# theEricMa/ScaleDreamer

Hardware: AMD Instinct MI355X
Metric: ASD train steps/sec (64x64 render, SD2.1) (higher is better)
Workload: dtype f32 renderer / f16 diffusion (f32 accumulate); 1 GPU; asd_sd_nerf: 1 view/GPU, 64x64 rays, 512 spp occgrid march, implicit-volume iNGP (16x2 hash grid 2^19, MLP 64), SD-2.1 UNet batch 5 (CFG+Perp-Neg+shifted t), VAE 512^2 fwd+bwd, AdamW; views_per_gpu=1, parallelism=dp1, diffusion_backend=hip, diffusion_weights=seeded random init (seed 1)

## Files before the change

### scaledreamer_amd/csrc/asd_common.h

```cpp
#pragma once
#include <hip/hip_runtime.h>
#include <stdint.h>

#include "../../include/asd_hip.h"

#define ASD_WAVE 64

void asd_set_error(const char* fmt, ...);

#define ASD_CHECK_ARG(cond, msg)                          \
    do {                                                  \
        if (!(cond)) {                                    \
            asd_set_error("%s: %s", __func__, msg);       \
            return ASD_ERR_ARG;                           \
        }                                                 \
    } while (0)

#define ASD_LAUNCH_CHECK()                                                         \
    do {                                                                           \
        hipError_t e__ = hipGetLastError();                                        \
        if (e__ != hipSuccess) {                                                   \
            asd_set_error("%s: launch failed: %s", __func__, hipGetErrorString(e__)); \
            return ASD_ERR_LAUNCH;                                                 \
        }                                                                          \
    } while (0)

static inline int asd_div_up(int64_t a, int64_t b) { return (int)((a + b - 1) / b); }

#include <atomic>
static inline bool asd_attr_needed(std::atomic<unsigned long long>& mask) {
    int dev = 0;
    (void)hipGetDevice(&dev);
    const unsigned long long bit = 1ull << (dev & 63);
    if (mask.load(std::memory_order_relaxed) & bit) return false;
    mask.fetch_or(bit, std::memory_order_relaxed);
    return true;
}

static inline int asd_grid_for(int64_t n, int block) {
    int g = asd_div_up(n, block);
    if (g < 1) g = 1;
    if (g > 2048) g = 2048;
    return g;
}

#ifdef __HIPCC__
__device__ __forceinline__ int asd_lane() { return (int)(threadIdx.x & 63); }

__device__ __forceinline__ float asd_wave_sum(float v) {
    int x;
#define ASD_DPP_ADD(CTRL, ROW_MASK)                                                                                      \
    x = __builtin_amdgcn_update_dpp(0, __float_as_int(v), CTRL, ROW_MASK, 0xf, true);                                    \
    v += __int_as_float(x)
    ASD_DPP_ADD(0x111, 0xf);
    ASD_DPP_ADD(0x112, 0xf);
    ASD_DPP_ADD(0x114, 0xf);
    ASD_DPP_ADD(0x118, 0xf);
    ASD_DPP_ADD(0x142, 0xa);
    ASD_DPP_ADD(0x143, 0xc);
#undef ASD_DPP_ADD
    return __int_as_float(__builtin_amdgcn_readlane(__float_as_int(v), 63));
}

__device__ __forceinline__ float asd_row_sum15(float v) {
    int x;
#define ASD_DPP_ADD(CTRL)                                                                                                \
    x = __builtin_amdgcn_update_dpp(0, __float_as_int(v), CTRL, 0xf, 0xf, true);                                         \
    v += __int_as_float(x)
    ASD_DPP_ADD(0x111);
    ASD_DPP_ADD(0x112);
    ASD_DPP_ADD(0x114);
    ASD_DPP_ADD(0x118);
#undef ASD_DPP_ADD
    return v;
}

__device__ __forceinline__ float asd_wave_incl_scan(float v) {
    const int lane = asd_lane();
#pragma unroll
    for (int o = 1; o < 64; o <<= 1) {
        const float u = __shfl_up(v, o, 64);
        if (lane >= o) v += u;
    }
    return v;
}
__device__ __forceinline__ float asd_wave_incl_prod(float v) {
    const int lane = asd_lane();
#pragma unroll
    for (int o = 1; o < 64; o <<= 1) {
        const float u = __shfl_up(v, o, 64);
        if (lane >= o) v *= u;
    }
    return v;
}
__device__ __forceinline__ int asd_ballot_rank(unsigned long long mask) {
    return (int)__builtin_amdgcn_mbcnt_hi((unsigned)(mask >> 32), __builtin_amdgcn_mbcnt_lo((unsigned)mask, 0u));
}

__device__ __forceinline__ float asd_softplus(float x) { return x > 20.f ? x : log1pf(expf(x)); }
__device__ __forceinline__ float asd_sigmoid(float x) { return 1.f / (1.f + expf(-x)); }
__device__ __forceinline__ float asd_clampf(float v, float lo, float hi) { return v < lo ? lo : (v > hi ? hi : v); }

__device__ __forceinline__ uint32_t asd_grid_index(const asd_grid_meta& m, int l, uint32_t cx, uint32_t cy,
                                                   uint32_t cz) {
    const uint32_t res = m.resolution[l];
    const uint32_t size = m.size[l];
    uint32_t di = cx + cy * res + cz * res * res;
    di -= (di >= size) ? size : 0u;
    const uint32_t hi = ((cx * 1u) ^ (cy * 2654435761u) ^ (cz * 805459861u)) & (size - 1u);
    return m.dense[l] ? di : hi;
}
__device__ __forceinline__ float asd_unit(float x) { return fminf(fmaxf(x, 0.f), 1.f); }

template <int L>
__device__ __forceinline__ void asd_encode(const asd_grid_meta& m, const float* __restrict__ params, float x,
                                           float y, float z, float (&enc)[2 * L]) {
    x = asd_unit(x); y = asd_unit(y); z = asd_unit(z);
#pragma unroll
    for (int l = 0; l < L; ++l) {
        const float s = m.scale[l];
        const float px = fmaf(s, x, 0.5f), py = fmaf(s, y, 0.5f), pz = fmaf(s, z, 0.5f);
        const float fx = floorf(px), fy = floorf(py), fz = floorf(pz);
        const uint32_t cx = (uint32_t)(int32_t)fx, cy = (uint32_t)(int32_t)fy, cz = (uint32_t)(int32_t)fz;
        const float wx = px - fx, wy = py - fy, wz = pz - fz;
        const float2* __restrict__ tab = reinterpret_cast<const float2*>(params) + m.offset[l];
        float2 v[8];
#pragma unroll
        for (int c = 0; c < 8; ++c)
            v[c] = tab[asd_grid_index(m, l, cx + (c & 1), cy + ((c >> 1) & 1), cz + ((c >> 2) & 1))];
        float f0 = 0.f, f1 = 0.f;
#pragma unroll
        for (int c = 0; c < 8; ++c) {
            const float ax = (c & 1) ? wx : 1.f - wx;
            const float ay = (c & 2) ? wy : 1.f - wy;
            const float az = (c & 4) ? wz : 1.f - wz;
            const float wt = ax * ay * az;
            f0 = fmaf(wt, v[c].x, f0);
            f1 = fmaf(wt, v[c].y, f1);
        }
        enc[2 * l] = f0;
        enc[2 * l + 1] = f1;
        if ((l & 3) == 3) __builtin_amdgcn_sched_barrier(0);
    }
}

template <int L>
__device__ __forceinline__ void asd_scatter(const asd_grid_meta& m, float* __restrict__ dparams, float x, float y,
                                            float z, const float (&denc)[2 * L]) {
    x = asd_unit(x); y = asd_unit(y); z = asd_unit(z);
#pragma unroll
    for (int l = 0; l < L; ++l) {
        const float g0 = denc[2 * l], g1 = denc[2 * l + 1];
        if (g0 == 0.f && g1 == 0.f) continue;
        const float s = m.scale[l];
        const float px = fmaf(s, x, 0.5f), py = fmaf(s, y, 0.5f), pz = fmaf(s, z, 0.5f);
        const float fx = floorf(px), fy = floorf(py), fz = floorf(pz);
        const uint32_t cx = (uint32_t)(int32_t)fx, cy = (uint32_t)(int32_t)fy, cz = (uint32_t)(int32_t)fz;
        const float wx = px - fx, wy = py - fy, wz = pz - fz;
        float* __restrict__ tab = dparams + 2u * (size_t)m.offset[l];
#pragma unroll
        for (int c = 0; c < 8; ++c) {
            const float ax = (c & 1) ? wx : 1.f - wx;
            const float ay = (c & 2) ? wy : 1.f - wy;
            const float az = (c & 4) ? wz : 1.f - wz;
            const float wt = ax * ay * az;
            const uint32_t idx = asd_grid_index(m, l, cx + (c & 1), cy + ((c >> 1) & 1), cz + ((c >> 2) & 1));
            atomicAdd(tab + 2u * (size_t)idx, wt * g0);
            atomicAdd(tab + 2u * (size_t)idx + 1, wt * g1);
        }
    }
}
#ifndef ASD_PRIV_COPIES
#define ASD_PRIV_COPIES 8
#endif
template <int L, int NAGG, int NPRIV = 0, bool FINE = true>
__device__ __forceinline__ void asd_scatter_runs(const asd_grid_meta& m, float* __restrict__ dparams, float x, float y,
                                                 float z, const float (&denc)[2 * L], bool active, float* __restrict__ priv = nullptr,
                                                 uint32_t priv_stride = 0) {
    static_assert(NPRIV <= NAGG, "only run-aggregated levels have per-XCD copies");
    x = asd_unit(x); y = asd_unit(y); z = asd_unit(z);
    const int lane = asd_lane();
    if (NPRIV > 0) {
        unsigned xcc, copy;
        asm volatile("s_getreg_b32 %0, hwreg(HW_REG_XCC_ID)" : "=s"(xcc));
        copy = xcc & 7u;
        if (ASD_PRIV_COPIES > 8) {
            unsigned hwid;
            asm volatile("s_getreg_b32 %0, hwreg(HW_REG_HW_ID)" : "=s"(hwid));
            copy = copy * (ASD_PRIV_COPIES / 8) + ((hwid >> 8) & (ASD_PRIV_COPIES / 8 - 1));
        }
        priv += (size_t)copy * priv_stride;
    }
#pragma unroll
    for (int l = 0; l < (NAGG < L ? NAGG : L); ++l) {
        const float g0 = active ? denc[2 * l] : 0.f, g1 = active ? denc[2 * l + 1] : 0.f;
        const float s = m.scale[l];
        const float px = fmaf(s, x, 0.5f), py = fmaf(s, y, 0.5f), pz = fmaf(s, z, 0.5f);
        const float fx = floorf(px), fy = floorf(py), fz = floorf(pz);
        const uint32_t cx = (uint32_t)(int32_t)fx, cy = (uint32_t)(int32_t)fy, cz = (uint32_t)(int32_t)fz;
        const float wx = px - fx, wy = py - fy, wz = pz - fz;
        float* __restrict__ tab = (l < NPRIV ? priv : dparams) + 2u * (size_t)m.offset[l];
        const uint32_t res = m.resolution[l];
        const uint32_t key = active ? cx + (cy + cz * res) * res : 0xFFFFFFFFu - (uint32_t)lane;
        const uint32_t prev = __shfl_up(key, 1, 64);
        const bool head = lane == 0 || prev != key;
        const unsigned long long hm = __ballot(head);
        const int rid = __popcll(hm & (~0ull >> (63 - lane)));
        float v[16];
#pragma unroll
        for (int c = 0; c < 8; ++c) {
            const float wt = ((c & 1) ? wx : 1.f - wx) * ((c & 2) ? wy : 1.f - wy) * ((c & 4) ? wz : 1.f - wz);
            v[2 * c] = wt * g0;
            v[2 * c + 1] = wt * g1;
        }
#pragma unroll
        for (int o = 1; o < 64; o <<= 1) {
            const int prid = __shfl_down(rid, o, 64);
            const bool ok = (lane + o < 64) && prid == rid;
#pragma unroll
            for (int q = 0; q < 16; ++q) {
                const float u = __shfl_down(v[q], o, 64);
                v[q] += ok ? u : 0.f;
            }
        }
        const bool issue = head && active;
        const bool carrier = !head && ((hm >> (lane - 1)) & 1ull);
        const bool self_f1 = issue && (lane == 63 || ((hm >> (lane + 1)) & 1ull));
#pragma unroll
        for (int c = 0; c < 8; ++c) {
            const uint32_t idx = asd_grid_index(m, l, cx + (c & 1), cy + ((c >> 1) & 1), cz + ((c >> 2) & 1));
            const float f1_prev = __shfl_up(v[2 * c + 1], 1, 64);
            const float val = issue ? v[2 * c] : f1_prev;
            float* dst = tab + 2u * (size_t)idx + (issue ? 0 : 1);
            if ((issue || carrier) && val != 0.f) atomicAdd(dst, val);
            if (self_f1 && v[2 * c + 1] != 0.f) atomicAdd(tab + 2u * (size_t)idx + 1, v[2 * c + 1]);
        }
    }
    if (NAGG >= L || !FINE) return;
    const int xb = (lane >> 1) & 1, ft = lane & 1;
#pragma unroll 1
    for (int q = 0; q < 4; ++q) {
        const int src = 16 * q + (lane >> 2);
        const float sx = __shfl(x, src, 64), sy = __shfl(y, src, 64), sz = __shfl(z, src, 64);
        const bool sact = __shfl((int)active, src, 64) != 0;
#pragma unroll
        for (int l = (NAGG < L ? NAGG : L); l < L; ++l) {
            const float ga = __shfl(denc[2 * l], src, 64), gb = __shfl(denc[2 * l + 1], src, 64);
            const float g = ft ? gb : ga;
            if (!sact || g == 0.f) continue;
            const float s = m.scale[l];
            const float px = fmaf(s, sx, 0.5f), py = fmaf(s, sy, 0.5f), pz = fmaf(s, sz, 0.5f);
            const float fx = floorf(px), fy = floorf(py), fz = floorf(pz);
            const uint32_t cx = (uint32_t)(int32_t)fx + (uint32_t)xb, cy = (uint32_t)(int32_t)fy, cz = (uint32_t)(int32_t)fz;
            const float wx = px - fx, wy = py - fy, wz = pz - fz;
            const float ax = xb ? wx : 1.f - wx;
            float* __restrict__ tab = dparams + 2u * (size_t)m.offset[l] + ft;
#pragma unroll
            for (int c = 0; c < 4; ++c) {
                const float wt = ax * ((c & 1) ? wy : 1.f - wy) * ((c & 2) ? wz : 1.f - wz);
                const uint32_t idx = asd_grid_index(m, l, cx, cy + (c & 1), cz + ((c >> 1) & 1));
                atomicAdd(tab + 2u * (size_t)idx, wt * g);
            }
        }
    }
}

extern hipEvent_t g_asd_probe_start, g_asd_probe_stop;
#define ASD_PROBE_START(s) do { if (g_asd_probe_start) (void)hipEventRecord(g_asd_probe_start, (s)); } while (0)
#define ASD_PROBE_STOP(s) do { if (g_asd_probe_stop) (void)hipEventRecord(g_asd_probe_stop, (s)); } while (0)

#endif
```

### scaledreamer_amd/csrc/gemm.hip

```cpp
#include <stdlib.h>

#include "asd_common.h"
#include <map>
#include <atomic>
#include <mutex>
#include <cstring>
#include <iterator>

#include "gemm_tile.h"


template <int BM, int BN, int WM, int WN, bool CONV, int NST = 2, int KG = 1, bool LN = false>
__global__ __launch_bounds__(WM * WN * KG * 64) void gemm_f16_kernel(const asd_gemm_args p) {
    constexpr int NW = WM * WN;
    constexpr int TM = BM / WM / 16, TN = BN / WN / 16;
    constexpr int RB = 128;
    constexpr int A_BYTES = BM * RB, B_BYTES = BN * RB;
    constexpr int STAGE_BYTES = A_BYTES + B_BYTES;
    constexpr int ASLABS = BM / 8, TSLABS = (BM + BN) / 8;
    constexpr int SPW = (TSLABS + NW - 1) / NW;
    static_assert(BM % (WM * 16) == 0 && BN % (WN * 16) == 0, "wave tile must be a multiple of 16 x 16");
    static_assert(NST == 2 || TSLABS % NW == 0, "ring variants count their loads per wave: every wave must own the same number of slabs");
    static_assert(KG == 1 || NST == 2, "k-groups use the two-stage loop");
    extern __shared__ __attribute__((aligned(16))) char smem[];

    const int tid = threadIdx.x, lane = tid & 63;
    const int wave_all = __builtin_amdgcn_readfirstlane(tid >> 6);
    const int kg = KG > 1 ? wave_all / NW : 0;
    const int wave = wave_all - kg * NW;
    char* const gsm = smem + kg * (NST * STAGE_BYTES);
    const int wm = wave / WN, wn = wave % WN;
    const bool up3 = CONV && p.upsample == 3;
    const int up_mq = up3 ? p.M >> 2 : 1;
    const int tiles_pp = (up_mq + BM - 1) / BM;
    const int tiles_m = up3 ? 4 * tiles_pp : (p.M + BM - 1) / BM, tiles_n = (p.N + BN - 1) / BN;
    int item, tm_, tn_;
    if (!asd_xcd_item(blockIdx.x, tiles_m * tiles_n * p.split_k, item)) return;
    const int kz = item / (tiles_m * tiles_n);
    asd_grouped_tile(item - kz * tiles_m * tiles_n, tiles_m, tiles_n, p.group_m, p.group_n, tm_, tn_);
    const int parity = up3 ? tm_ / tiles_pp : 0;
    const int m0 = up3 ? parity * up_mq + (tm_ - parity * tiles_pp) * BM : tm_ * BM, n0 = tn_ * BN;
    const int m_lim = up3 ? (parity + 1) * up_mq : p.M;
    const int k_steps_total = (p.K + 63) / 64;
    const int k_per = (k_steps_total + p.split_k - 1) / p.split_k;
    const int ks0 = kz * k_per, ks1 = min(k_steps_total, ks0 + k_per);

    const int lrow = lane >> 3, pchunk = lane & 7;
    const char* zero = (const char*)p.zero_page;
    const bool fast_conv = CONV && (p.upsample == 0 || p.upsample == 3) && (p.Cin & 63) == 0;
    const int par_a = parity >> 1, par_b = parity & 1;
    const char* const Wp = (const char*)p.W + ((CONV && p.upsample == 3) ? (size_t)parity * p.N * p.ldw * 2 : 0);
    const int lch = pchunk ^ lrow;
    constexpr int ASPW = (ASLABS + NW - 1) / NW;
    const char* a0 = nullptr;
    const char* c_base[CONV ? ASPW : 1];
    int c_yx[CONV ? ASPW : 1];
    if (!CONV) {
        a0 = (const char*)p.A + (size_t)(m0 + lrow) * p.lda * 2 + lch * 16;
    } else {
#pragma unroll
        for (int j = 0; j < ASPW; ++j) {
            const int slab = wave + j * NW;
            int m = min(m0 + slab * 8 + lrow, m_lim - 1);
            int hw = p.Hout * p.Wout, wrow = p.Wout;
            if (p.upsample == 3) { m -= parity * up_mq; hw = p.Hin * p.Win; wrow = p.Win; }
            const int b = m / hw, r = m - b * hw;
            int y = r / wrow, x = r - y * wrow;
            c_base[j] = (const char*)p.A + (size_t)b * p.Hin * p.Win * p.Cin * 2;
            if (fast_conv) {
                y *= p.stride; x *= p.stride;
                c_base[j] += ((size_t)(y * p.Win + x) * p.Cin) * 2 + lch * 16;
            }
            c_yx[j] = (y << 16) | x;
        }
    }
    constexpr bool WIDE_OK = (BN / WN) % 32 == 0;
    const bool wide = WIDE_OK && p.wide_rows;
    const int wl = wide ? wide_lane_row(lrow) : lrow;
    auto w_slab_rows = [&](int ws) { return wide ? wide_slab_rows(ws) : ws * 8; };
    const char* w0 = Wp + (size_t)(n0 + wl) * p.ldw * 2 + lch * 16;
    const size_t a_slab_stride = (size_t)8 * p.lda * 2, w_row_stride = (size_t)p.ldw * 2;
    unsigned roff[SPW];
#pragma unroll
    for (int j = 0; j < SPW; ++j) {
        const int slab = wave + j * NW;
        if (slab >= ASLABS) {
            const int row = min(n0 + w_slab_rows(slab - ASLABS) + wl, p.N - 1);
            roff[j] = (unsigned)row * (unsigned)(p.ldw * 2) + lch * 16 + (ks0 + kg) * 128;
            if (!CONV && p.w_seg_rows > 0) {
                const int seg = row / p.w_seg_rows;
                roff[j] = (unsigned)(row - seg * p.w_seg_rows) * (unsigned)(p.ldw * 2) + (unsigned)p.w_seg_off[seg] + lch * 16 + (ks0 + kg) * 128;
            }
        } else {
            const int row = min(m0 + slab * 8 + lrow, p.M - 1);
            roff[j] = CONV ? 0u : (unsigned)row * (unsigned)(p.lda * 2) + lch * 16 + (ks0 + kg) * 128;
            if (!CONV && p.a_seg_rows > 0) {
                const int seg = row / p.a_seg_rows;
                roff[j] = (unsigned)(row - seg * p.a_seg_rows) * (unsigned)(p.lda * 2) + (unsigned)p.a_seg_off[seg] + lch * 16 + (ks0 + kg) * 128;
            }
        }
    }

    auto issue_rows = [&](int stage) __attribute__((always_inline)) {
        char* st = gsm + stage * STAGE_BYTES;
#pragma unroll
        for (int j = 0; j < SPW; ++j) {
            const int slab = wave + j * NW;
            if (j * NW + NW - 1 >= TSLABS && slab >= TSLABS) continue;
            if (CONV && slab < ASLABS) continue;
            const char* base = slab >= ASLABS ? Wp : (const char*)p.A;
            load_slab(base + roff[j], st + slab * 8 * RB);
            roff[j] += 128 * KG;
        }
    };
    auto issue_general = [&](int ks, int stage, bool only_conv_a) __attribute__((always_inline)) {
        char* st = gsm + stage * STAGE_BYTES;
        const int k0 = ks * 64;
        const int kc = k0 + lch * 8;
        const bool k_ok = kc < p.K;
        int opaque = 0;
        asm volatile("" : "+v"(opaque));
        int tdy = 0, tdx = 0;
        long long toff = 0;
        if (fast_conv) {
            const int tap = k0 / p.Cin, c0 = k0 - tap * p.Cin;
            if (p.upsample == 3) { tdy = (tap >> 1) - 1 + par_a; tdx = (tap & 1) - 1 + par_b; }
            else { const int ky = tap / 3, kx = tap - ky * 3; tdy = ky - p.pad; tdx = kx - p.pad; }
            toff = ((long long)(tdy * p.Win + tdx) * p.Cin + c0) * 2;
        }
#pragma unroll
        for (int j = 0; j < SPW; ++j) {
            const int slab = wave + j * NW;
            if (slab >= TSLABS) continue;
            if (only_conv_a && slab >= ASLABS) continue;
            const char* src;
            if (slab >= ASLABS) {
                const int ws = slab - ASLABS;
                const int wr = w_slab_rows(ws);
                src = (k_ok && n0 + wr + wl < p.N) ? w0 + (wr + opaque) * w_row_stride + (size_t)k0 * 2 : zero;
            } else if (!CONV) {
                src = (k_ok && m0 + slab * 8 + lrow < p.M) ? a0 + (slab + opaque) * a_slab_stride + (size_t)k0 * 2 : zero;
            } else {
                constexpr int JA = CONV ? ASPW : 1;
                const int ja = j < JA ? j : JA - 1;
                const bool row_ok = m0 + slab * 8 + lrow < m_lim;
                const int sy = c_yx[ja] >> 16, sx = c_yx[ja] & 0xffff;
                if (fast_conv) {
                    const int yi = sy + tdy, xi = sx + tdx;
                    const bool ok = row_ok && (unsigned)yi < (unsigned)p.Hin && (unsigned)xi < (unsigned)p.Win;
                    src = ok ? c_base[ja] + toff : zero;
                } else {
                    const int tap = kc / p.Cin, c0 = kc - tap * p.Cin;
                    const int ky = tap / 3, kx = tap - ky * 3;
                    int yi = sy * p.stride + ky - p.pad, xi = sx * p.stride + kx - p.pad;
                    bool ok = row_ok && k_ok;
                    if (p.upsample == 3) {
                        yi = sy + (tap >> 1) - 1 + par_a; xi = sx + (tap & 1) - 1 + par_b;
                        ok = ok && yi >= 0 && xi >= 0 && yi < p.Hin && xi < p.Win;
                    } else if (p.upsample == 1) {
                        ok = ok && yi >= 0 && xi >= 0 && yi < 2 * p.Hin && xi < 2 * p.Win;
                        yi >>= 1; xi >>= 1;
                    } else if (p.upsample == 2) {
                        yi = sy + p.pad - ky; xi = sx + p.pad - kx;
                        ok = ok && yi >= 0 && xi >= 0 && !(yi & 1) && !(xi & 1) && (yi >> 1) < p.Hin && (xi >> 1) < p.Win;
                        yi >>= 1; xi >>= 1;
                    } else {
                        ok = ok && yi >= 0 && xi >= 0 && yi < p.Hin && xi < p.Win;
                    }
                    src = ok ? c_base[ja] + ((size_t)(yi * p.Win + xi) * p.Cin + c0) * 2 : zero;
                }
            }
            load_slab(src, st + slab * 8 * RB);
        }
    };
    auto issue = [&](int ks, int stage) __attribute__((always_inline)) {
        if (ks * 64 + 64 > p.K || (CONV && !fast_conv)) {
            issue_general(ks, stage, false);
        } else {
            issue_rows(stage);
            if (CONV) issue_general(ks, stage, true);
        }
    };

    floatx4 acc[TM][TN];
#pragma unroll
    for (int i = 0; i < TM; ++i)
#pragma unroll
        for (int j = 0; j < TN; ++j) acc[i][j] = floatx4{0.f, 0.f, 0.f, 0.f};
    floatx4 sacc[LN ? TM : 1], qacc[LN ? TM : 1];
#pragma unroll
    for (int i = 0; i < (LN ? TM : 1); ++i) sacc[i] = qacc[i] = floatx4{0.f, 0.f, 0.f, 0.f};
    const half8 ln_ones = {(half_t)1.f, (half_t)1.f, (half_t)1.f, (half_t)1.f, (half_t)1.f, (half_t)1.f, (half_t)1.f, (half_t)1.f};
    float ls1[LN ? TM : 1], ls2[LN ? TM : 1];
    auto ln_extract = [&]() __attribute__((always_inline)) {
        if constexpr (LN) {
            const int b = lane & 15;
#pragma unroll
            for (int i = 0; i < TM; ++i) {
                ls1[i] = sacc[i][0];
                const float d = (b & 2) ? ((b & 1) ? qacc[i][3] : qacc[i][2]) : ((b & 1) ? qacc[i][1] : qacc[i][0]);
                ls2[i] = __shfl(d, b + 16 * (b >> 2), 64);
            }
        }
    };

    const int frow = lane & 15, fq = lane >> 4;
    const int fa0 = (wm * (BM / WM) + frow) * RB, fb0 = A_BYTES + (wn * (BN / WN) + frow) * RB;
    const int fsw[2] = {((fq) ^ (frow & 7)) * 16, ((4 + fq) ^ (frow & 7)) * 16};

    int live_ky_parity = -1;
    if (NST == 2 && KG == 1 && CONV && p.upsample == 2 && (p.Cin & 63) == 0) {
        const int m_last = min(m0 + BM, p.M) - 1;
        if (m0 / p.Wout == m_last / p.Wout) live_ky_parity = ((m0 / p.Wout) % p.Hout + p.pad) & 1;
    }
    auto live = [&](int ks) -> bool {
        if (!CONV || live_ky_parity < 0) return true;
        const int ky = ((ks * 64) / p.Cin) / 3;
        return (ky & 1) == live_ky_parity;
    };
    auto compute = [&](const char* As) __attribute__((always_inline)) {
#pragma unroll TM * TN >= 32 ? 1 : 2
        for (int kh = 0; kh < 2; ++kh) {
            half8 xa[TM], wb[TN];
            const int fs = TM * TN >= 32 ? (((kh * 4 + fq) ^ (frow & 7)) * 16) : fsw[kh];
#pragma unroll
            for (int i = 0; i < TM; ++i) xa[i] = *(const half8*)(As + fa0 + fs + i * 16 * RB);
#pragma unroll
            for (int j = 0; j < TN; ++j) wb[j] = *(const half8*)(As + fb0 + fs + j * 16 * RB);
#pragma unroll
            for (int i = 0; i < TM; ++i)
#pragma unroll
                for (int j = 0; j < TN; ++j)
                    acc[i][j] = __builtin_amdgcn_mfma_f32_16x16x32_f16(wb[j], xa[i], acc[i][j], 0, 0, 0);
            if constexpr (LN) {
#pragma unroll
                for (int i = 0; i < TM; ++i) {
                    sacc[i] = __builtin_amdgcn_mfma_f32_16x16x32_f16(ln_ones, xa[i], sacc[i], 0, 0, 0);
                    qacc[i] = __builtin_amdgcn_mfma_f32_16x16x32_f16(xa[i], xa[i], qacc[i], 0, 0, 0);
                }
            }
        }
    };
    if constexpr (KG > 1) {
        int k = ks0 + kg;
        const int iters = (ks1 - ks0 + KG - 1) / KG;
        if (k < ks1) issue(k, 0);
        for (int it = 0, stage = 0; it < iters; ++it, stage ^= 1) {
            asm volatile("s_waitcnt vmcnt(0)" ::: "memory");
            __builtin_amdgcn_s_barrier();
            const int kn = k + KG;
            if (kn < ks1) issue(kn, stage ^ 1);
            if (k < ks1) compute(gsm + stage * STAGE_BYTES);
            k = kn;
        }
        ln_extract();
        floatx4* red = (floatx4*)smem;
#pragma unroll 1
        for (int g = KG - 1; g >= 1; --g) {
            __syncthreads();
            if (kg == g) {
#pragma unroll
                for (int i = 0; i < TM; ++i)
#pragma unroll
                    for (int j = 0; j < TN; ++j) red[((wave * TM + i) * TN + j) * 64 + lane] = acc[i][j];
            }
            __syncthreads();
            if (kg == 0) {
#pragma unroll
                for (int i = 0; i < TM; ++i)
#pragma unroll
                    for (int j = 0; j < TN; ++j) {
                        const floatx4 t = red[((wave * TM + i) * TN + j) * 64 + lane];
                        acc[i][j][0] += t[0]; acc[i][j][1] += t[1]; acc[i][j][2] += t[2]; acc[i][j][3] += t[3];
                    }
            }
            if constexpr (LN) {
                float* redf = (float*)(red + NW * TM * TN * 64);
                __syncthreads();
                if (kg == g) {
#pragma unroll
                    for (int i = 0; i < TM; ++i) { redf[((wave * TM + i) * 2) * 64 + lane] = ls1[i]; redf[((wave * TM + i) * 2 + 1) * 64 + lane] = ls2[i]; }
                }
                __syncthreads();
                if (kg == 0) {
#pragma unroll
                    for (int i = 0; i < TM; ++i) { ls1[i] += redf[((wave * TM + i) * 2) * 64 + lane]; ls2[i] += redf[((wave * TM + i) * 2 + 1) * 64 + lane]; }
                }
            }
        }
    } else if constexpr (NST > 2) {
        const int nk = ks1 - ks0;
        if (nk > 0) {
#pragma unroll
            for (int s = 0; s < NST - 1; ++s)
                if (s < nk) issue(ks0 + s, s);
            int stage = 0, fill = NST - 1;
            for (int i = 0; i < nk; ++i) {
                ring_wait<SPW, NST - 2>(nk - 1 - i);
                __builtin_amdgcn_s_barrier();
                if (i + NST - 1 < nk) issue(ks0 + i + NST - 1, fill);
                compute(gsm + stage * STAGE_BYTES);
                stage = stage + 1 == NST ? 0 : stage + 1;
                fill = fill + 1 == NST ? 0 : fill + 1;
            }
        }
    } else {
    int k = ks0;
    while (k < ks1 && !live(k)) ++k;
    if (k < ks1) {
        issue(k, 0);
        for (int stage = 0;; stage ^= 1) {
            asm volatile("s_waitcnt vmcnt(0)" ::: "memory");
            __builtin_amdgcn_s_barrier();
            int kn = k + 1;
            while (kn < ks1 && !live(kn)) ++kn;
            if (kn < ks1) issue(kn, stage ^ 1);
            compute(gsm + stage * STAGE_BYTES);
            if (kn >= ks1) break;
            k = kn;
        }
    }
    }
    if constexpr (KG == 1) ln_extract();

    const int em = lane & 15, en = (lane >> 4) * 4;
    auto out_row = [&](int i) {
        const int m = m0 + wm * (BM / WM) + i * 16 + em;
        if (m >= m_lim) return -1;
        if (CONV && p.upsample == 3) {
            const int q = m - parity * up_mq, hwq = p.Hin * p.Win;
            const int bb = q / hwq, r = q - bb * hwq, y = r / p.Win, x = r - y * p.Win;
            return (bb * p.Hout + 2 * y + par_a) * p.Wout + 2 * x + par_b;
        }
        return m;
    };
    if (KG > 1 && kg != 0) {
        if (p.split_k == 1 && p.act != 2 && p.gn_partials != nullptr) {
            __syncthreads(); __syncthreads();
            __syncthreads();
        }
        return;
    }
    if (p.split_k > 1) {
        tile_epilogue<TM, TN>(p, acc, n0 + wn * (BN / WN), kz, m0, out_row, false, nullptr);
        return;
    }
    float ln_mean[LN ? TM : 1], ln_rstd[LN ? TM : 1];
    if constexpr (LN) {
        const float inv_k = 1.f / (float)p.K;
#pragma unroll
        for (int i = 0; i < TM; ++i) {
            ln_mean[i] = ls1[i] * inv_k;
            ln_rstd[i] = rsqrtf(fmaxf(ls2[i] * inv_k - ln_mean[i] * ln_mean[i], 0.f) + p.ln_eps);
            const int m = m0 + wm * (BM / WM) + i * 16 + em;
            if (p.ln_stats && n0 == 0 && wn == 0 && lane < 16 && m < p.M) { p.ln_stats[2 * m] = ln_mean[i]; p.ln_stats[2 * m + 1] = ln_rstd[i]; }
        }
    }
    if (p.act == 2) {
        if constexpr (TN % 2 == 0) {
#pragma unroll
            for (int i = 0; i < TM; ++i) {
                const int m = m0 + wm * (BM / WM) + i * 16 + em;
                if (m >= p.M) continue;
#pragma unroll
                for (int j = 0; j < TN; j += 2) {
                    const int n = n0 + wn * (BN / WN) + j * 16 + en;
                    if (n + 16 >= p.N) continue;
                    const half4 bx = *(const half4*)((const half_t*)p.bias + n), bg = *(const half4*)((const half_t*)p.bias + n + 16);
                    float va[4] = {acc[i][j][0], acc[i][j][1], acc[i][j][2], acc[i][j][3]};
                    float vg[4] = {acc[i][j + 1][0], acc[i][j + 1][1], acc[i][j + 1][2], acc[i][j + 1][3]};
                    if (p.ln_mode) {
                        ln_fold<4>(p, va, m, n, LN ? ln_mean[i] : 0.f, LN ? ln_rstd[i] : 0.f);
                        ln_fold<4>(p, vg, m, n + 16, LN ? ln_mean[i] : 0.f, LN ? ln_rstd[i] : 0.f);
                    }
                    half4 o;
#pragma unroll
                    for (int r = 0; r < 4; ++r)
                        o[r] = (half_t)((va[r] + (float)bx[r]) * gelu_erf(vg[r] + (float)bg[r]));
                    *(half4*)((half_t*)p.C + (size_t)m * p.ldc + (n >> 5) * 16 + (n & 15)) = o;
                }
            }
        }
        return;
    }
    const bool gn = p.gn_partials != nullptr;
    float* gn_lds = (float*)smem;
    if (gn) gn_tile_begin(gn_lds);
    tile_epilogue<TM, TN>(p, acc, n0 + wn * (BN / WN), kz, m0, out_row, gn, gn_lds, LN ? ln_mean : nullptr, LN ? ln_rstd : nullptr);
    if (gn) gn_tile_end(p, gn_lds, (m0 / BM) * ((p.N + BN - 1) / BN) + n0 / BN);
}

#define LDS_READ16(dst, addr, OFF) asm volatile("ds_read_b128 %0, %1 offset:%2" : "=&v"(dst) : "v"(addr), "n"(OFF) : "memory")
#define LGKM_WAIT(N, F)                                                                                                  \
    asm volatile("s_waitcnt lgkmcnt(" #N ")"                                                                             \
                 : "+v"(F.a[0]), "+v"(F.a[1]), "+v"(F.a[2]), "+v"(F.a[3]), "+v"(F.w[0]), "+v"(F.w[1]), "+v"(F.w[2]), "+v"(F.w[3]))

template <int BN>
__global__ __launch_bounds__(512) void conv3x3_win_kernel(const asd_gemm_args p) {
    constexpr int WN = 2, TM = 4, TN = BN / WN / 16;
    constexpr int RB = 128;
    constexpr int WIN = 18, WIN_ROWS = WIN * WIN, WIN_SLABS = (WIN_ROWS + 7) / 8;
    constexpr int A_BYTES = WIN_SLABS * 8 * RB, W_BYTES = BN * RB;
    constexpr int WSLABS = BN / 8, WSPW = (WSLABS + 7) / 8;
    extern __shared__ __attribute__((aligned(16))) char smem[];
    char* const a_buf = smem;
    char* const w_buf = smem + 2 * A_BYTES;

    const int tid = threadIdx.x, lane = tid & 63, wave = tid >> 6;
    const int wm = wave >> 1, wn = wave & 1;
    const int tiles_x = p.Wout / 16, tiles_y = p.Hout / 16;
    const int tiles_m = (p.M / (p.Hout * p.Wout)) * tiles_y * tiles_x;
    const int tiles_n = (p.N + BN - 1) / BN;
    int item, tm, tn_;
    if (!asd_xcd_item(blockIdx.x, tiles_m * tiles_n * p.split_k, item)) return;
    const int kz = item / (tiles_m * tiles_n);
    asd_grouped_tile(item - kz * tiles_m * tiles_n, tiles_m, tiles_n, p.group_m, p.group_n, tm, tn_);
    const int n0 = tn_ * BN;
    const int b = tm / (tiles_y * tiles_x), tr = tm - b * tiles_y * tiles_x;
    const int y0 = (tr / tiles_x) * 16, x0 = (tr - (tr / tiles_x) * tiles_x) * 16;
    const int n_chunks = p.Cin / 64;
    const int c_per = (n_chunks + p.split_k - 1) / p.split_k;
    const int c0 = kz * c_per, c1 = min(n_chunks, c0 + c_per);
    const int steps = (c1 - c0) * 9;

    const int lrow = lane >> 3, pchunk = lane & 7;
    const char* zero = (const char*)p.zero_page;
    const char* img = (const char*)p.A + (size_t)b * p.Hin * p.Win * p.Cin * 2;
    const bool wide = p.wide_rows != 0;
    const int wl = wide ? wide_lane_row(lrow) : lrow;
    const char* w0 = (const char*)p.W + (size_t)(n0 + wl) * p.ldw * 2 + (pchunk ^ lrow) * 16;
    const size_t w_row_stride = (size_t)p.ldw * 2;

    auto load_window_slab = [&](int slab, int chunk, char* dst_buf) {
        const int wrow = slab * 8 + lrow;
        const int wy = (wrow * 3641) >> 16, wx = wrow - wy * WIN;
        const int yi = y0 - 1 + wy, xi = x0 - 1 + wx;
        const bool ok = wrow < WIN_ROWS && (unsigned)yi < (unsigned)p.Hin && (unsigned)xi < (unsigned)p.Win;
        const char* src = ok ? img + ((size_t)(yi * p.Win + xi) * p.Cin + chunk * 64) * 2 + (pchunk ^ (wx & 7)) * 16 : zero;
        load_slab(src, dst_buf + slab * 8 * RB);
    };
    auto load_w_tile = [&](int step, char* dst_buf) {
        const int chunk = c0 + step / 9, tap = step - (step / 9) * 9;
        const size_t koff = ((size_t)tap * p.Cin + chunk * 64) * 2;
#pragma unroll
        for (int j = 0; j < WSPW; ++j) {
            const int slab = wave + j * 8;
            if (slab >= WSLABS) continue;
            const int wr = wide ? wide_slab_rows(slab) : slab * 8;
            const char* src = (n0 + wr + wl < p.N) ? w0 + wr * w_row_stride + koff : zero;
            load_slab(src, dst_buf + slab * 8 * RB);
        }
    };

    floatx4 acc[TM][TN];
#pragma unroll
    for (int i = 0; i < TM; ++i)
#pragma unroll
        for (int j = 0; j < TN; ++j) acc[i][j] = floatx4{0.f, 0.f, 0.f, 0.f};

    const int frow = lane & 15, fq = lane >> 4;
    const unsigned lds_a = (unsigned)(size_t)a_buf + (unsigned)((wm * 4 * WIN + frow) * RB);
    const unsigned lds_w = (unsigned)(size_t)w_buf + (unsigned)((wn * (BN / WN) + frow) * RB);
    const unsigned fsww[2] = {(unsigned)(((fq) ^ (frow & 7)) * 16), (unsigned)(((4 + fq) ^ (frow & 7)) * 16)};
    struct Frag { half8 a[4], w[4]; };
    static_assert(TM == 4 && (TN == 4 || TN == 2), "fragment sets are written for 4 x {2, 4} sub-tiles");

    auto read_frags = [&](Frag& f, int s, int kh) {
        const int cl = s / 9, tap = s - cl * 9;
        const int ky = tap / 3, kx = tap - ky * 3;
        const unsigned aa = lds_a + (unsigned)((cl & 1) * A_BYTES + (ky * WIN + kx) * RB) + (unsigned)(((kh * 4 + fq) ^ ((frow + kx) & 7)) * 16);
        const unsigned wa = lds_w + (unsigned)((s & 3) * W_BYTES) + fsww[kh];
        LDS_READ16(f.a[0], aa, 0 * WIN * RB);
        LDS_READ16(f.a[1], aa, 1 * WIN * RB);
        LDS_READ16(f.a[2], aa, 2 * WIN * RB);
        LDS_READ16(f.a[3], aa, 3 * WIN * RB);
        LDS_READ16(f.w[0], wa, 0 * 16 * RB);
        LDS_READ16(f.w[1], wa, 1 * 16 * RB);
        if constexpr (TN == 4) {
            LDS_READ16(f.w[2], wa, 2 * 16 * RB);
            LDS_READ16(f.w[3], wa, 3 * 16 * RB);
        } else {
            f.w[2] = f.w[0]; f.w[3] = f.w[1];
        }
    };
    auto mma = [&](const Frag& f) {
#pragma unroll
        for (int i = 0; i < TM; ++i)
#pragma unroll
            for (int j = 0; j < TN; ++j)
                acc[i][j] = __builtin_amdgcn_mfma_f32_16x16x32_f16(f.w[j], f.a[i], acc[i][j], 0, 0, 0);
    };
    constexpr int NRD = TM + TN;

    if (steps > 0) {
        for (int slab = wave; slab < WIN_SLABS; slab += 8) load_window_slab(slab, c0, a_buf);
        load_w_tile(0, w_buf);
        if (steps > 1) load_w_tile(1, w_buf + W_BYTES);
        Frag f0, f1;
#pragma unroll 1
        for (int s = 0; s < steps; s += 2) {
            const int cl = s / 9;
            asm volatile("s_waitcnt vmcnt(0)" ::: "memory");
            __builtin_amdgcn_s_barrier();
            if (s + 2 < steps) load_w_tile(s + 2, w_buf + ((s + 2) & 3) * W_BYTES);
            if (s + 3 < steps) load_w_tile(s + 3, w_buf + ((s + 3) & 3) * W_BYTES);
            if (c0 + cl + 1 < c1 && s > 9 * cl) {
                const int base = ((s - 9 * cl - 1) >> 1) * 16;
#pragma unroll
                for (int h = 0; h < 2; ++h) {
                    const int slab = base + h * 8 + wave;
                    if (slab < WIN_SLABS) load_window_slab(slab, c0 + cl + 1, a_buf + ((cl + 1) & 1) * A_BYTES);
                }
            }
            const bool two = s + 1 < steps;
            read_frags(f0, s, 0);
            read_frags(f1, s, 1);
            if constexpr (NRD == 8) LGKM_WAIT(8, f0); else LGKM_WAIT(6, f0);
            mma(f0);
            __builtin_amdgcn_sched_barrier(0);
            if (two) {
                read_frags(f0, s + 1, 0);
                if constexpr (NRD == 8) LGKM_WAIT(8, f1); else LGKM_WAIT(6, f1);
                mma(f1);
                __builtin_amdgcn_sched_barrier(0);
                read_frags(f1, s + 1, 1);
                if constexpr (NRD == 8) LGKM_WAIT(8, f0); else LGKM_WAIT(6, f0);
                mma(f0);
                __builtin_amdgcn_sched_barrier(0);
                LGKM_WAIT(0, f1);
                mma(f1);
            } else {
                LGKM_WAIT(0, f1);
                mma(f1);
            }
            __builtin_amdgcn_sched_barrier(0);
        }
    }

    const bool gn = p.gn_partials != nullptr && p.split_k == 1;
    float* gn_lds = (float*)smem;
    if (gn) gn_tile_begin(gn_lds);
    tile_epilogue<TM, TN>(p, acc, n0 + wn * (BN / WN), kz, b * p.Hout * p.Wout,
                          [&](int i) { return (b * p.Hout + y0 + wm * 4 + i) * p.Wout + x0 + frow; }, gn, gn_lds);
    if (gn) gn_tile_end(p, gn_lds, tm * tiles_n + tn_);
}

template <int BN, int NW = 8>
__global__ __launch_bounds__(NW * 64, NW / 2) void conv3x3_win2_kernel(const asd_gemm_args p) {
    constexpr int WN = NW / 4, TM = 4, TN = BN / WN / 16;
    constexpr int RB = 128;
    constexpr int WIN = 18, WIN_ROWS = WIN * WIN, WIN_SLABS = (WIN_ROWS + 7) / 8;
    constexpr int A_BYTES = WIN_SLABS * 8 * RB, W_BYTES = BN * RB;
    constexpr int WSLABS = BN / 8, WSPW = (WSLABS + NW - 1) / NW;
    extern __shared__ __attribute__((aligned(16))) char smem[];
    char* const a_buf = smem;
    char* const w_buf = smem + A_BYTES;

    const int tid = threadIdx.x, lane = tid & 63, wave = __builtin_amdgcn_readfirstlane(tid >> 6);
    const int wm = wave / WN, wn = wave - wm * WN;
    const int tiles_x = p.Wout / 16, tiles_y = p.Hout / 16;
    const int tiles_m = (p.M / (p.Hout * p.Wout)) * tiles_y * tiles_x;
    const int tiles_n = (p.N + BN - 1) / BN;
    int item, tm, tn_;
    if (!asd_xcd_item(blockIdx.x, tiles_m * tiles_n * p.split_k, item)) return;
    const int kz = item / (tiles_m * tiles_n);
    asd_grouped_tile(item - kz * tiles_m * tiles_n, tiles_m, tiles_n, p.group_m, p.group_n, tm, tn_);
    const int n0 = tn_ * BN;
    const int b = tm / (tiles_y * tiles_x), tr = tm - b * tiles_y * tiles_x;
    const int y0 = (tr / tiles_x) * 16, x0 = (tr - (tr / tiles_x) * tiles_x) * 16;
    const int n_chunks = p.Cin / 64;
    const int c_per = (n_chunks + p.split_k - 1) / p.split_k;
    const int c0 = kz * c_per, c1 = min(n_chunks, c0 + c_per);
    const int steps = (c1 - c0) * 9;

    const int lrow = lane >> 3, pchunk = lane & 7, lch = pchunk ^ lrow;
    const char* zero = (const char*)p.zero_page;
    const char* img = (const char*)p.A + (size_t)b * p.Hin * p.Win * p.Cin * 2;
    const bool wide = p.wide_rows != 0;
    const int wl = wide ? wide_lane_row(lrow) : lrow;
    const char* w0 = (const char*)p.W + (size_t)(n0 + wl) * p.ldw * 2 + lch * 16;
    const size_t w_row_stride = (size_t)p.ldw * 2;

    auto load_window_slab = [&](int slab, int chunk, char* dst_buf) {
        const int wrow = slab * 8 + lrow;
        const int wy = (wrow * 3641) >> 16, wx = wrow - wy * WIN;
        const int yi = y0 - 1 + wy, xi = x0 - 1 + wx;
        const bool ok = wrow < WIN_ROWS && (unsigned)yi < (unsigned)p.Hin && (unsigned)xi < (unsigned)p.Win;
        const char* src = ok ? img + ((size_t)(yi * p.Win + xi) * p.Cin + chunk * 64) * 2 + (pchunk ^ (wx & 7)) * 16 : zero;
        load_slab(src, dst_buf + slab * 8 * RB);
    };
    auto load_w_tile = [&](int step, char* dst_buf) {
        const int chunk = c0 + step / 9, tap = step - (step / 9) * 9;
        const size_t koff = ((size_t)tap * p.Cin + chunk * 64) * 2;
#pragma unroll
        for (int j = 0; j < WSPW; ++j) {
            const int slab = wave + j * NW;
            if (slab >= WSLABS) continue;
            const int wr = wide ? wide_slab_rows(slab) : slab * 8;
            const char* src = (n0 + wr + wl < p.N) ? w0 + wr * w_row_stride + koff : zero;
            load_slab(src, dst_buf + slab * 8 * RB);
        }
    };

    floatx4 acc[TM][TN];
#pragma unroll
    for (int i = 0; i < TM; ++i)
#pragma unroll
        for (int j = 0; j < TN; ++j) acc[i][j] = floatx4{0.f, 0.f, 0.f, 0.f};

    const int frow = lane & 15, fq = lane >> 4;
    const int fb0 = (wn * (BN / WN) + frow) * RB;
    const int fswb[2] = {((fq) ^ (frow & 7)) * 16, ((4 + fq) ^ (frow & 7)) * 16};

#ifdef ASD_WIN_PROFILE
    unsigned long long pt_start = __builtin_amdgcn_s_memtime(), pt_wait = 0, pt_first = 0, pt_reload = 0, pt_loop_end = 0;
#define PT_NOW() __builtin_amdgcn_s_memtime()
#endif
    if (steps > 0) {
        for (int slab = wave; slab < WIN_SLABS; slab += NW) load_window_slab(slab, c0, a_buf);
        load_w_tile(0, w_buf);
#pragma unroll 1
        for (int s = 0; s < steps; ++s) {
            const int cl = s / 9, tap = s - cl * 9;
#ifdef ASD_WIN_PROFILE
            const unsigned long long pt_a = PT_NOW();
#endif
            if (tap == 0 && s > 0) {
                __builtin_amdgcn_s_barrier();
                for (int slab = wave; slab < WIN_SLABS; slab += NW) load_window_slab(slab, c0 + cl, a_buf);
            }
            asm volatile("s_waitcnt vmcnt(0)" ::: "memory");
            __builtin_amdgcn_s_barrier();
#ifdef ASD_WIN_PROFILE
            {
                const unsigned long long pt_b = PT_NOW();
                if (s == 0) pt_first = pt_b - pt_a; else if (tap == 0) pt_reload += pt_b - pt_a; else pt_wait += pt_b - pt_a;
            }
#endif
            if (s + 1 < steps) load_w_tile(s + 1, w_buf + ((s + 1) & 1) * W_BYTES);
            const char* Wt = w_buf + (s & 1) * W_BYTES;
            const int ky = tap / 3, kx = tap - ky * 3;
            const char* Ar = a_buf + ((wm * 4 + ky) * WIN + frow + kx) * RB;
            const int csw = (frow + kx) & 7;
            if constexpr (NW == 4) {
                half8 xa[2][TM], wb[2][TN];
#pragma unroll
                for (int kh = 0; kh < 2; ++kh) {
                    const char* Ak = Ar + (((kh * 4 + fq) ^ csw) * 16);
#pragma unroll
                    for (int i = 0; i < TM; ++i) xa[kh][i] = *(const half8*)(Ak + i * WIN * RB);
#pragma unroll
                    for (int j = 0; j < TN; ++j) wb[kh][j] = *(const half8*)(Wt + fb0 + fswb[kh] + j * 16 * RB);
                }
                __builtin_amdgcn_sched_barrier(0);
#pragma unroll
                for (int kh = 0; kh < 2; ++kh)
#pragma unroll
                    for (int i = 0; i < TM; ++i)
#pragma unroll
                        for (int j = 0; j < TN; ++j)
                            acc[i][j] = __builtin_amdgcn_mfma_f32_16x16x32_f16(wb[kh][j], xa[kh][i], acc[i][j], 0, 0, 0);
            } else {
#pragma unroll
            for (int kh = 0; kh < 2; ++kh) {
                half8 xa[TM], wb[TN];
                const char* Ak = Ar + (((kh * 4 + fq) ^ csw) * 16);
#pragma unroll
                for (int i = 0; i < TM; ++i) xa[i] = *(const half8*)(Ak + i * WIN * RB);
#pragma unroll
                for (int j = 0; j < TN; ++j) wb[j] = *(const half8*)(Wt + fb0 + fswb[kh] + j * 16 * RB);
#pragma unroll
                for (int i = 0; i < TM; ++i)
#pragma unroll
                    for (int j = 0; j < TN; ++j)
                        acc[i][j] = __builtin_amdgcn_mfma_f32_16x16x32_f16(wb[j], xa[i], acc[i][j], 0, 0, 0);
            }
            }
        }
    }

#ifdef ASD_WIN_PROFILE
    pt_loop_end = PT_NOW();
#endif
    const bool gn = p.gn_partials != nullptr && p.split_k == 1;
    float* gn_lds = (float*)smem;
    if (gn) gn_tile_begin(gn_lds);
    tile_epilogue<TM, TN>(p, acc, n0 + wn * (BN / WN), kz, b * p.Hout * p.Wout,
                          [&](int i) { return (b * p.Hout + y0 + wm * 4 + i) * p.Wout + x0 + frow; }, gn, gn_lds);
    if (gn) gn_tile_end(p, gn_lds, tm * tiles_n + tn_);
#ifdef ASD_WIN_PROFILE
    if (p.split_k == 1 && p.workspace && lane == 0) {
        asm volatile("s_waitcnt vmcnt(0)" ::: "memory");
        unsigned long long* o = (unsigned long long*)p.workspace + ((size_t)item * NW + wave) * 8;
        o[0] = pt_start; o[1] = PT_NOW(); o[2] = pt_first; o[3] = pt_wait; o[4] = pt_reload; o[5] = pt_loop_end;
        unsigned hwid; asm volatile("s_getreg_b32 %0, hwreg(HW_REG_HW_ID)" : "=s"(hwid));
        unsigned xcc; asm volatile("s_getreg_b32 %0, hwreg(HW_REG_XCC_ID)" : "=s"(xcc));
        o[6] = hwid; o[7] = xcc;
    }
#endif
}

__global__ __launch_bounds__(256) void splitk_epilogue_kernel(const asd_gemm_args p, int splits) {
    const size_t q = (size_t)blockIdx.x * 256 + threadIdx.x;
    const size_t total4 = (size_t)p.M * p.N / 4;
    if (q >= total4) return;
    const int m = (int)((q * 4) / p.N), n = (int)((q * 4) % p.N);
    floatx4 v = {0.f, 0.f, 0.f, 0.f};
    for (int s = 0; s < splits; ++s) {
        const floatx4 t = *(const floatx4*)(p.workspace + ((size_t)s * p.M + m) * p.N + n);
        v[0] += t[0]; v[1] += t[1]; v[2] += t[2]; v[3] += t[3];
    }
    if (p.bias) {
        const half4 b = *(const half4*)((const half_t*)p.bias + n);
        v[0] += (float)b[0]; v[1] += (float)b[1]; v[2] += (float)b[2]; v[3] += (float)b[3];
    }
    if (p.row_bias) {
        const half4 b = *(const half4*)((const half_t*)p.row_bias + (size_t)(m / p.rows_per_group) * p.ld_row_bias + n);
        v[0] += (float)b[0]; v[1] += (float)b[1]; v[2] += (float)b[2]; v[3] += (float)b[3];
    }
    if (p.act == 1) {
#pragma unroll
        for (int r = 0; r < 4; ++r) v[r] = v[r] / (1.f + __expf(-v[r]));
    }
    if (p.residual) {
        const half4 b = *(const half4*)((const half_t*)p.residual + (size_t)m * p.ldr + n);
        v[0] += (float)b[0]; v[1] += (float)b[1]; v[2] += (float)b[2]; v[3] += (float)b[3];
    }
    if (p.out_f32) {
        *(floatx4*)((float*)p.C + (size_t)m * p.ldc + n) = v;
    } else {
        half4 o = {(half_t)v[0], (half_t)v[1], (half_t)v[2], (half_t)v[3]};
        *(half4*)((half_t*)p.C + (size_t)m * p.ldc + n) = o;
    }
}

__global__ __launch_bounds__(256) void splitk_epilogue_gn_kernel(const asd_gemm_args p, int splits) {
    __shared__ float lds64[64];
    const int tiles_n = p.N / 64;
    const int mb = blockIdx.x / tiles_n, nb = blockIdx.x - mb * tiles_n;
    const int tx = threadIdx.x & 15, ty = threadIdx.x >> 4;
    const int n = nb * 64 + tx * 4;
    if (threadIdx.x < 64) lds64[threadIdx.x] = 0.f;
    __syncthreads();
    floatx4 cs = {0.f, 0.f, 0.f, 0.f}, cq = {0.f, 0.f, 0.f, 0.f};
    half4 bias = {0, 0, 0, 0};
    if (p.bias) bias = *(const half4*)((const half_t*)p.bias + n);
    floatx4 v[4];
    int mrow[4];
#pragma unroll
    for (int i = 0; i < 4; ++i) {
        v[i] = floatx4{0.f, 0.f, 0.f, 0.f};
        mrow[i] = min(mb * 64 + i * 16 + ty, p.M - 1);
    }
    for (int s = 0; s < splits; ++s) {
        floatx4 t[4];
#pragma unroll
        for (int i = 0; i < 4; ++i) t[i] = *(const floatx4*)(p.workspace + ((size_t)s * p.M + mrow[i]) * p.N + n);
#pragma unroll
        for (int i = 0; i < 4; ++i) { v[i][0] += t[i][0]; v[i][1] += t[i][1]; v[i][2] += t[i][2]; v[i][3] += t[i][3]; }
    }
#pragma unroll
    for (int i = 0; i < 4; ++i) {
        const int m = mb * 64 + i * 16 + ty;
        if (m >= p.M) continue;
        floatx4 w = v[i];
        w[0] += (float)bias[0]; w[1] += (float)bias[1]; w[2] += (float)bias[2]; w[3] += (float)bias[3];
        if (p.row_bias) {
            const half4 b = *(const half4*)((const half_t*)p.row_bias + (size_t)(m / p.rows_per_group) * p.ld_row_bias + n);
            w[0] += (float)b[0]; w[1] += (float)b[1]; w[2] += (float)b[2]; w[3] += (float)b[3];
        }
        if (p.act == 1) {
#pragma unroll
            for (int r = 0; r < 4; ++r) w[r] = w[r] / (1.f + __expf(-w[r]));
        }
        if (p.residual) {
            const half4 b = *(const half4*)((const half_t*)p.residual + (size_t)m * p.ldr + n);
            w[0] += (float)b[0]; w[1] += (float)b[1]; w[2] += (float)b[2]; w[3] += (float)b[3];
        }
        const half4 o = {(half_t)w[0], (half_t)w[1], (half_t)w[2], (half_t)w[3]};
        *(half4*)((half_t*)p.C + (size_t)m * p.ldc + n) = o;
#pragma unroll
        for (int r = 0; r < 4; ++r) { const float f = (float)o[r]; cs[r] += f; cq[r] = fmaf(f, f, cq[r]); }
    }
#pragma unroll
    for (int r = 0; r < 4; ++r) {
        const int g = (n + r) / p.gn_cg;
        atomicAdd(&lds64[2 * g], cs[r]);
        atomicAdd(&lds64[2 * g + 1], cq[r]);
    }
    __syncthreads();
    if (threadIdx.x < 64) p.gn_partials[(size_t)blockIdx.x * 64 + threadIdx.x] = lds64[threadIdx.x];
}

#define GNA_THREADS 1024
template <int NV>
__global__ __launch_bounds__(GNA_THREADS) void splitk_epilogue_gnapply_kernel(const asd_gemm_args p, int splits) {
    __shared__ float red[2 * (GNA_THREADS / 64)];
    const int cg = p.gn_cg, g4 = cg >> 2, rows = p.gn_rows;
    const int b = blockIdx.x >> 5, g = blockIdx.x & 31;
    const int n0 = g * cg, total = rows * g4, tid = threadIdx.x;
    floatx4 v[NV];
    int mrow[NV], ncol[NV];
#pragma unroll
    for (int i = 0; i < NV; ++i) {
        const int e = min(tid + GNA_THREADS * i, total - 1);
        const int r = e / g4;
        mrow[i] = b * rows + r;
        ncol[i] = n0 + (e - r * g4) * 4;
        v[i] = floatx4{0.f, 0.f, 0.f, 0.f};
    }
    half4 bias[NV], rbias[NV], resid[NV];
#pragma unroll
    for (int i = 0; i < NV; ++i) {
        const int m = mrow[i], n = ncol[i];
        bias[i] = p.bias ? *(const half4*)((const half_t*)p.bias + n) : half4{0, 0, 0, 0};
        rbias[i] = p.row_bias ? *(const half4*)((const half_t*)p.row_bias + (size_t)(m / p.rows_per_group) * p.ld_row_bias + n) : half4{0, 0, 0, 0};
        resid[i] = p.residual ? *(const half4*)((const half_t*)p.residual + (size_t)m * p.ldr + n) : half4{0, 0, 0, 0};
    }
    for (int s = 0; s < splits; s += 4) {
        floatx4 t[4][NV];
#pragma unroll
        for (int u = 0; u < 4; ++u) {
            const int su = min(s + u, splits - 1);
#pragma unroll
            for (int i = 0; i < NV; ++i) t[u][i] = *(const floatx4*)(p.workspace + ((size_t)su * p.M + mrow[i]) * p.N + ncol[i]);
        }
#pragma unroll
        for (int u = 0; u < 4; ++u) {
            const float on = s + u < splits ? 1.f : 0.f;
#pragma unroll
            for (int i = 0; i < NV; ++i) {
                v[i][0] = fmaf(t[u][i][0], on, v[i][0]); v[i][1] = fmaf(t[u][i][1], on, v[i][1]);
                v[i][2] = fmaf(t[u][i][2], on, v[i][2]); v[i][3] = fmaf(t[u][i][3], on, v[i][3]);
            }
        }
    }
    float cs = 0.f, cq = 0.f;
#pragma unroll
    for (int i = 0; i < NV; ++i) {
        const int m = mrow[i], n = ncol[i];
        floatx4 w = v[i];
#pragma unroll
        for (int r = 0; r < 4; ++r) w[r] += (float)bias[i][r];
#pragma unroll
        for (int r = 0; r < 4; ++r) w[r] += (float)rbias[i][r];
        if (p.act == 1) {
#pragma unroll
            for (int r = 0; r < 4; ++r) w[r] = w[r] / (1.f + __expf(-w[r]));
        }
#pragma unroll
        for (int r = 0; r < 4; ++r) w[r] += (float)resid[i][r];
        const half4 o = {(half_t)w[0], (half_t)w[1], (half_t)w[2], (half_t)w[3]};
        const bool live = tid + GNA_THREADS * i < total;
        if (live) *(half4*)((half_t*)p.C + (size_t)m * p.ldc + n) = o;
#pragma unroll
        for (int r = 0; r < 4; ++r) {
            const float f = (float)o[r];
            v[i][r] = f;
            if (live) { cs += f; cq = fmaf(f, f, cq); }
        }
    }
#pragma unroll
    for (int off = 32; off > 0; off >>= 1) { cs += __shfl_xor(cs, off, 64); cq += __shfl_xor(cq, off, 64); }
    if ((tid & 63) == 0) { red[(tid >> 6) * 2] = cs; red[(tid >> 6) * 2 + 1] = cq; }
    __syncthreads();
    float sum = 0.f, sq = 0.f;
#pragma unroll
    for (int w = 0; w < GNA_THREADS / 64; ++w) { sum += red[2 * w]; sq += red[2 * w + 1]; }
    if (p.gn_apply_stats && tid == 0) { p.gn_apply_stats[b * 64 + g * 2] = sum; p.gn_apply_stats[b * 64 + g * 2 + 1] = sq; }
    const float inv_cnt = 1.f / ((float)rows * (float)cg);
    const float mean = sum * inv_cnt;
    const float var = fmaxf(sq * inv_cnt - mean * mean, 0.f);
    const float rstd = rsqrtf(var + p.gn_apply_eps);
#pragma unroll
    for (int i = 0; i < NV; ++i) {
        if (tid + GNA_THREADS * i >= total) continue;
        const int m = mrow[i], n = ncol[i];
        const half4 gm = *(const half4*)((const half_t*)p.gn_apply_gamma + n), bt = *(const half4*)((const half_t*)p.gn_apply_beta + n);
        half4 o;
#pragma unroll
        for (int r = 0; r < 4; ++r) {
            const float sa = rstd * (float)gm[r];
            float f = fmaf(v[i][r], sa, (float)bt[r] - mean * sa);
            if (p.gn_apply_silu) f = f / (1.f + __expf(-f));
            o[r] = (half_t)f;
        }
        *(half4*)((half_t*)p.gn_apply_y + (size_t)m * p.N + n) = o;
    }
}

#define ASD_GNAPPLY_MAX_NV 5
static int asd_gemm_gn_apply_nv(const asd_gemm_args* a) {
    if (!a->gn_apply || a->split_k <= 1 || a->partials_only || a->out_f32 || a->act == 2 || a->gn_bwd_x) return 0;
    if (a->gn_cg < 4 || a->gn_cg % 4 || a->N != 32 * a->gn_cg || a->gn_rows < 1 || a->M % a->gn_rows || a->ldc % 4) return 0;
    if (a->conv && a->upsample == 3) return 0;
    const int need = (a->gn_rows * (a->gn_cg / 4) + GNA_THREADS - 1) / GNA_THREADS;
    static const int max_nv = getenv("ASD_GNAPPLY_MAX_NV") ? atoi(getenv("ASD_GNAPPLY_MAX_NV")) : 3;
    if (need > max_nv) return 0;
    return need <= 1 ? 1 : need <= 3 ? 3 : need <= ASD_GNAPPLY_MAX_NV ? ASD_GNAPPLY_MAX_NV : 0;
}

static void asd_launch_splitk_epilogue(const asd_gemm_args* a, hipStream_t s) {
    const int nv = a->gn_apply_y ? asd_gemm_gn_apply_nv(a) : 0;
    if (nv > 0) {
        const dim3 grid((a->M / a->gn_rows) * 32);
        if (nv == 1) hipLaunchKernelGGL(splitk_epilogue_gnapply_kernel<1>, grid, dim3(GNA_THREADS), 0, s, *a, a->split_k);
        else if (nv == 3) hipLaunchKernelGGL(splitk_epilogue_gnapply_kernel<3>, grid, dim3(GNA_THREADS), 0, s, *a, a->split_k);
        else hipLaunchKernelGGL(splitk_epilogue_gnapply_kernel<ASD_GNAPPLY_MAX_NV>, grid, dim3(GNA_THREADS), 0, s, *a, a->split_k);
        return;
    }
    const size_t total4 = (size_t)a->M * a->N / 4;
    if (a->gn_partials) hipLaunchKernelGGL(splitk_epilogue_gn_kernel, dim3((a->M / 64) * (a->N / 64)), dim3(256), 0, s, *a, a->split_k);
    else hipLaunchKernelGGL(splitk_epilogue_kernel, dim3(asd_div_up(total4, 256)), dim3(256), 0, s, *a, a->split_k);
}


struct asd_gemm_tile { int bm, bn, wm, wn, nst, kg; };
#define ASD_GEMM_NCFG 29
#define ASD_GEMM_WIN0 8
#define ASD_GEMM_PP0 20
static const asd_gemm_tile asd_gemm_tiles[ASD_GEMM_NCFG] = {
    {128, 64, 2, 2}, {128, 128, 2, 2}, {256, 64, 4, 2}, {256, 128, 4, 2}, {128, 320, 2, 4}, {256, 256, 2, 4}, {256, 320, 2, 4},
    {320, 128, 5, 2}, {256, 64, 4, 2}, {256, 128, 4, 2}, {256, 64, 4, 2}, {256, 128, 4, 2},
    {64, 64, 2, 2},
    {256, 64, 4, 1}, {256, 128, 4, 1},
    {64, 64, 2, 2, 4, 1}, {64, 64, 2, 2, 2, 2}, {64, 64, 2, 2, 2, 4}, {128, 64, 2, 2, 2, 2}, {128, 128, 2, 2, 2, 2},
    {512, 128, 4, 2}, {256, 256, 4, 2}, {256, 320, 4, 2}, {256, 128, 4, 2}, {256, 160, 4, 2},
    {320, 64, 2, 2},
    {128, 64, 2, 2, 6, 1}, {64, 64, 2, 2, 8, 1}, {128, 128, 2, 2, 4, 1}};
#define ASD_GEMM_WS 25
static int asd_cfg_stages(int cfg) { return asd_gemm_tiles[cfg].nst > 2 ? asd_gemm_tiles[cfg].nst : 2; }
static int asd_cfg_kgroups(int cfg) { return asd_gemm_tiles[cfg].kg > 1 ? asd_gemm_tiles[cfg].kg : 1; }
static bool asd_cfg_is_pp(int cfg) { return cfg >= ASD_GEMM_PP0 && cfg < ASD_GEMM_PP0 + 5; }
static bool asd_cfg_is_window(int cfg) { return (cfg >= ASD_GEMM_WIN0 && cfg < ASD_GEMM_WIN0 + 4) || cfg == 13 || cfg == 14 || asd_cfg_is_pp(cfg); }
static bool asd_cfg_is_win2(int cfg) { return cfg == ASD_GEMM_WIN0 + 2 || cfg == ASD_GEMM_WIN0 + 3 || cfg == 13 || cfg == 14; }
static bool asd_cfg_is_ws(int cfg) { return cfg == ASD_GEMM_WS; }
int asd_conv_ws_launch(const asd_gemm_args* a, hipStream_t s);
static bool asd_conv_ws_ok(const asd_gemm_args* a) {
    return a->conv && a->stride == 1 && a->pad == 1 && a->upsample == 0 && a->Hin == 8 && a->Win == 8 && a->Hout == 8 && a->Wout == 8 &&
           a->M % 64 == 0 && a->M / 64 <= 5 && a->N % 64 == 0 && a->split_k >= 2 && a->Cin % (32 * a->split_k) == 0 && !a->gn_bwd_x && !a->ln_mode;
}
size_t asd_conv_pp_lds_bytes(int variant);
int asd_conv_pp_launch(int variant, const asd_gemm_args* a, int blocks, hipStream_t s);

static bool asd_conv_window_ok(const asd_gemm_args* a) {
    return a->conv && a->stride == 1 && a->pad == 1 && a->upsample == 0 && a->Cin % 64 == 0 && a->Hin == a->Hout &&
           a->Win == a->Wout && a->Hout % 16 == 0 && a->Wout % 16 == 0;
}

static bool asd_conv_pp_ok(const asd_gemm_args* a, int cfg) {
    return a->conv && a->stride == 1 && a->pad == 1 && a->upsample == 0 && a->Cin % 32 == 0 && a->Hin == a->Hout && a->Win == a->Wout &&
           a->Hout % 16 == 0 && a->Wout % 16 == 0 && a->Hout % (asd_gemm_tiles[cfg].bm / 16) == 0 && a->N % asd_gemm_tiles[cfg].bn == 0;
}
static int g_force_tile = -1;

static int asd_gemm_pick_tile(int M, int N, int K, int split) {
    const int ksteps = asd_div_up(asd_div_up(K, 64), split);
    double best = 1e300;
    int best_cfg = 1;
    for (int c = 0; c < ASD_GEMM_WIN0; ++c) {
        const int bm = asd_gemm_tiles[c].bm, bn = asd_gemm_tiles[c].bn;
        if (bn > 64 && N % bn != 0 && !(bn == 128 && N % 128 == 0)) continue;
        if (bn == 64 && N % 128 == 0) continue;
        const long long blocks = (long long)asd_div_up(M, bm) * asd_div_up(N, bn) * split;
        const double per_block = (double)ksteps * (bm + bn) + 6.0 * 64 + 0.02 * bm * bn;
        const double rounds = blocks >= 256 ? (double)blocks / 256.0 : 0.62 + 0.38 * (double)blocks / 256.0;
        const double cost = per_block * rounds;
        if (cost < best) { best = cost; best_cfg = c; }
    }
    return best_cfg;
}

struct asd_plan_key {
    int32_t M, N, K, conv, a, b, c, d, e;
    bool operator<(const asd_plan_key& o) const { return memcmp(this, &o, sizeof(*this)) < 0; }
};
struct asd_plan_val { int32_t tile, split; };
static std::map<asd_plan_key, asd_plan_val> g_plans;
static std::mutex g_plans_mu;
static std::atomic<uint64_t> g_plan_gen{1};

static asd_plan_key asd_plan_key_of(const asd_gemm_args* a) {
    asd_plan_key k;
    memset(&k, 0, sizeof(k));
    k.M = a->M; k.N = a->N; k.K = a->K; k.conv = a->conv ? 1 : 0;
    if (a->conv) { k.a = a->Hin; k.b = a->Cin; k.c = a->stride; k.d = a->upsample; k.e = a->pad; }
    else k.a = a->act == 2 ? -a->lda : a->lda;
    return k;
}
static bool asd_plan_lookup(const asd_gemm_args* a, asd_plan_val* out) {
    std::lock_guard<std::mutex> lk(g_plans_mu);
    auto it = g_plans.find(asd_plan_key_of(a));
    if (it == g_plans.end()) return false;
    *out = it->second;
    return true;
}
static int asd_default_split(const asd_gemm_args* a) {
    if (a->act == 2) return 1;
    const int bn = a->N % 128 == 0 ? 128 : 64;
    const int tiles = asd_div_up(a->M, 128) * asd_div_up(a->N, bn);
    if (tiles >= 256 || a->K < 1024) return 1;
    const int target = tiles <= 128 ? 512 : 640;
    int s = target / tiles;
    if (s > 16) s = 16;
    if (s > a->K / 512) s = a->K / 512;
    return s < 1 ? 1 : s;
}

__global__ void asd_touch_kernel(const uint4* __restrict__ p, size_t n16, unsigned* __restrict__ sink) {
    unsigned acc = 0;
    for (size_t i = (size_t)blockIdx.x * blockDim.x + threadIdx.x; i < n16; i += (size_t)gridDim.x * blockDim.x) {
        const uint4 v = p[i];
        acc ^= v.x ^ v.y ^ v.z ^ v.w;
    }
    if (acc == 0x9e3779b9u) sink[0] = acc;
}

__global__ void asd_spin_kernel(long long cycles) {
    const long long t0 = wall_clock64();
    while (wall_clock64() - t0 < cycles) {}
}

static int asd_gemm_resolve_cfg(const asd_gemm_args* a) {
    int cfg = asd_gemm_pick_tile(a->M, a->N, a->K, a->split_k);
    if (asd_conv_window_ok(a) && a->M >= 4096 && a->split_k <= a->Cin / 64) {
        cfg = a->N % 128 == 0 ? 9 : 8;
        if ((a->M / 256) * asd_div_up(a->N, asd_gemm_tiles[cfg].bn) * a->split_k >= 512) cfg += 2;
    }
    if (a->act == 2 && (cfg == 4 || cfg == 6)) cfg = a->N % 256 == 0 ? 5 : (a->N % 128 == 0 ? 3 : 2);
    if (a->tile_cfg >= 1 && a->tile_cfg <= ASD_GEMM_NCFG) cfg = a->tile_cfg - 1;
    if (g_force_tile >= 0 && g_force_tile < ASD_GEMM_NCFG) cfg = g_force_tile;
    if (a->conv && a->upsample == 3 && asd_cfg_is_window(cfg)) cfg = a->N % 128 == 0 ? 1 : 0;
    return cfg;
}

#define ASD_SPLITK_GN_MAX_RECORDS 96
static int asd_gemm_gn_records_cfg(const asd_gemm_args* a, int cfg, bool need_ptr) {
    if (a->gn_bwd_x && !(a->gn_bwd_fstats && a->gn_bwd_gamma && a->gn_bwd_beta && a->ldc == a->N)) return 0;
    if ((need_ptr && !a->gn_partials) || a->split_k < 1 || a->out_f32 || a->act == 2 || a->gn_cg < 1 || a->gn_rows < 1 || a->N != 32 * a->gn_cg || a->M % a->gn_rows) return 0;
    if (a->conv && a->upsample == 3) return 0;
    if (a->split_k > 1) {
        if (a->gn_bwd_x || a->N % 64 || a->gn_rows % 64 || a->ldc % 4) return 0;
        const int nrec = (a->gn_rows / 64) * (a->N / 64);
        return nrec <= ASD_SPLITK_GN_MAX_RECORDS ? nrec : 0;
    }
    const int bn = asd_gemm_tiles[cfg].bn, tiles_n = asd_div_up(a->N, bn);
    if (asd_cfg_is_window(cfg)) return a->gn_rows % asd_gemm_tiles[cfg].bm == 0 ? (a->gn_rows / asd_gemm_tiles[cfg].bm) * tiles_n : 0;
    const int bm = asd_gemm_tiles[cfg].bm;
    return a->gn_rows % bm == 0 ? (a->gn_rows / bm) * tiles_n : 0;
}

extern "C" {

int asd_gemm_force_tile(int32_t cfg) {
    g_force_tile = cfg;
    ++g_plan_gen;
    return ASD_OK;
}

int asd_gemm_plan_set(int32_t M, int32_t N, int32_t K, int32_t conv, int32_t s0, int32_t s1, int32_t s2, int32_t s3, int32_t s4,
                      int32_t tile_cfg, int32_t split_k) {
    ASD_CHECK_ARG(tile_cfg >= 0 && tile_cfg <= ASD_GEMM_NCFG && split_k >= 1, "bad plan");
    asd_plan_key k;
    memset(&k, 0, sizeof(k));
    k.M = M; k.N = N; k.K = K; k.conv = conv ? 1 : 0; k.a = s0; k.b = s1; k.c = s2; k.d = s3; k.e = s4;
    std::lock_guard<std::mutex> lk(g_plans_mu);
    g_plans[k] = asd_plan_val{tile_cfg, split_k};
    ++g_plan_gen;
    return ASD_OK;
}

int asd_gemm_plan_get(const asd_gemm_args* a, int32_t* tile_cfg, int32_t* split_k) {
    ASD_CHECK_ARG(a && tile_cfg && split_k, "null argument");
    asd_plan_val v;
    if (asd_plan_lookup(a, &v)) { *tile_cfg = v.tile; *split_k = v.split; return ASD_OK; }
    *tile_cfg = 0;
    *split_k = asd_default_split(a);
    return 1;
}

int32_t asd_gemm_gn_records(const asd_gemm_args* a_in) {
    if (!a_in || a_in->M <= 0 || a_in->N <= 0 || a_in->K <= 0) return 0;
    asd_gemm_args a = *a_in;
    if (a.split_k == 0) {
        int32_t t = 0, sk = 1;
        asd_gemm_plan_get(&a, &t, &sk);
        a.split_k = sk;
        if (a.tile_cfg == 0) a.tile_cfg = t;
    }
    return asd_gemm_gn_records_cfg(&a, asd_gemm_resolve_cfg(&a), false);
}

int32_t asd_gemm_gn_applies(const asd_gemm_args* a_in) {
    if (!a_in || a_in->M <= 0 || a_in->N <= 0 || a_in->K <= 0) return 0;
    asd_gemm_args a = *a_in;
    if (a.split_k == 0) {
        int32_t t = 0, sk = 1;
        asd_gemm_plan_get(&a, &t, &sk);
        a.split_k = sk;
    }
    return asd_gemm_gn_apply_nv(&a) > 0 ? 1 : 0;
}

int asd_gemm_plan_count(void) {
    std::lock_guard<std::mutex> lk(g_plans_mu);
    return (int)g_plans.size();
}

int64_t asd_gemm_workspace_bytes(const asd_gemm_args* a) {
    int32_t t = 0, s = 1;
    if (!a) return 0;
    if (a->split_k >= 1) s = a->split_k; else asd_gemm_plan_get(a, &t, &s);
    return s > 1 ? (int64_t)s * a->M * a->N * 4 : 0;
}

static void asd_pick_group(int tiles_m, int tiles_n, int bm, int bn, size_t lds, int* gm, int* gn) {
    const int conc = 32 * (2 * lds <= 160 * 1024 ? 2 : 1);
    int m = (int)lroundf(sqrtf((float)conc * (float)bn / (float)bm));
    m = m < 1 ? 1 : (m > tiles_m ? tiles_m : m);
    int n = conc / m;
    n = n < 1 ? 1 : (n > tiles_n ? tiles_n : n);
    if (n == tiles_n) { m = conc / n; m = m < 1 ? 1 : (m > tiles_m ? tiles_m : m); }
    *gm = m; *gn = n;
}

int asd_gemm_f16(const asd_gemm_args* a_in, void* stream) {
    ASD_CHECK_ARG(a_in, "null argument");
    asd_gemm_args a_copy = *a_in;
    asd_gemm_args* a = &a_copy;
    if (a->ld_row_bias <= 0) a->ld_row_bias = a->N;
    if (a->split_k == 0) {
        int32_t t = 0, sk = 1;
        asd_gemm_plan_get(a, &t, &sk);
        a->split_k = sk;
        if (a->tile_cfg == 0) a->tile_cfg = t;
    }
    ASD_CHECK_ARG(a && a->A && a->W && a->C && a->zero_page, "null argument");
    ASD_CHECK_ARG(a->M > 0 && a->N > 0 && a->K > 0, "empty problem");
    ASD_CHECK_ARG(a->K % 8 == 0, "K must be a multiple of 8");
    ASD_CHECK_ARG(a->N % 4 == 0 && a->ldc % 4 == 0, "N and ldc must be multiples of 4");
    ASD_CHECK_ARG(a->ldw % 8 == 0 && (a->conv || a->lda % 8 == 0), "leading dimensions must be multiples of 8 halfs (16 B)");
    if (a->conv) {
        ASD_CHECK_ARG(a->Cin % 8 == 0 && a->K == (a->upsample == 3 ? 4 : 9) * a->Cin, "conv: Cin must be a multiple of 8 and K = 9*Cin (4*Cin in the parity form)");
        ASD_CHECK_ARG(a->upsample != 3 || (a->stride == 1 && a->Hout == 2 * a->Hin && a->Wout == 2 * a->Win && !a->gn_bwd_x),
                      "parity-form upsample conv: stride 1, Hout = 2*Hin, Wout = 2*Win");
        ASD_CHECK_ARG(a->Hout > 0 && a->Wout > 0 && a->M % (a->Hout * a->Wout) == 0, "conv: M must be B*Hout*Wout");
    }
    ASD_CHECK_ARG(a->split_k >= 1 && (a->split_k == 1 || a->workspace), "split-K needs a workspace");
    if (a->a_seg_rows > 0 || a->w_seg_rows > 0 || a->partials_only)
        ASD_CHECK_ARG(!a->conv && a->K % 64 == 0 && a->a_seg_rows >= 0 && a->w_seg_rows >= 0 && (!a->partials_only || a->split_k > 1) &&
                      (a->a_seg_rows == 0 || (a->M + a->a_seg_rows - 1) / a->a_seg_rows <= 9) && (a->w_seg_rows == 0 || (a->N + a->w_seg_rows - 1) / a->w_seg_rows <= 6),
                      "segmented rows / partials_only: plain GEMM, K % 64 == 0, at most 9 (A) and 6 (W) segments, split_k > 1 for partials_only");
    ASD_CHECK_ARG((size_t)a->N * a->ldw * 2 < ((size_t)1 << 32) && (a->conv || (size_t)a->M * a->lda * 2 < ((size_t)1 << 32)),
                  "row-major operands are addressed with 32-bit byte offsets (< 4 GiB each)");
    if (a->act == 2)
        ASD_CHECK_ARG(a->N % 32 == 0 && a->bias && !a->conv && !a->residual && !a->row_bias && !a->out_f32 && a->split_k == 1,
                      "GEGLU epilogue: N % 32 == 0, bias required, no conv / residual / row_bias / fp32 output / split-K");
    if (a->ln_mode) {
        ASD_CHECK_ARG((a->ln_mode == 1 || a->ln_mode == 2) && a->ln_sc && !a->out_f32, "LayerNorm fold: ln_mode 1 | 2, ln_sc required, fp16 output");
        ASD_CHECK_ARG(a->ln_mode == 1 || (a->ln_stats && a->N % 4 == 0), "LayerNorm fold, mode 2: the column statistics ln_stats[N][2] are required");
        ASD_CHECK_ARG(a->ln_mode == 2 || !a->conv, "LayerNorm fold, mode 1: plain GEMM only (the rows of A are the LayerNorm's rows)");
        if (a->split_k > 1) { a->split_k = 1; a->tile_cfg = 0; }
    }
    int cfg = asd_gemm_resolve_cfg(a);
    ASD_CHECK_ARG(a->act != 2 || (!asd_cfg_is_window(cfg) && (asd_gemm_tiles[cfg].bn / asd_gemm_tiles[cfg].wn) % 32 == 0),
                  "GEGLU epilogue needs a tile whose per-wave width is a multiple of 32 columns");
    ASD_CHECK_ARG(asd_gemm_tiles[cfg].bn == 64 || a->N % asd_gemm_tiles[cfg].bn == 0 || (asd_gemm_tiles[cfg].bn == 128 && a->N % 4 == 0),
                  "tile configuration does not divide N");
    const int bm = asd_gemm_tiles[cfg].bm, bn = asd_gemm_tiles[cfg].bn;
    if (asd_gemm_gn_records_cfg(a, cfg, true) == 0) a->gn_partials = nullptr;
    {
        static const bool wide_on = !(getenv("ASD_WIDE_ROWS") && getenv("ASD_WIDE_ROWS")[0] == '0');
        auto al16 = [](const void* q) { return ((uintptr_t)q & 15) == 0; };
        const int wave_n = bn / asd_gemm_tiles[cfg].wn;
        a->wide_rows = wide_on && wave_n % 32 == 0 && a->act != 2 && a->N % 8 == 0 && a->ldc % 8 == 0 && al16(a->C) && (!a->bias || al16(a->bias)) &&
                       (!a->row_bias || (al16(a->row_bias) && a->ld_row_bias % 8 == 0)) && (!a->residual || (al16(a->residual) && a->ldr % 8 == 0)) &&
                       !(a->gn_partials && a->gn_bwd_x);
    }
    static const bool trace = getenv("ASD_GEMM_TRACE") != nullptr;
    if (trace)
        fprintf(stderr, "ASD_GEMM %d %d %d conv=%d %d %d %d %d %d s=%d p=%d u=%d cfg=%d split=%d act=%d res=%d f32=%d gn=%d\n", a->M, a->N, a->K, a->conv, a->Hin,
                a->Win, a->Cin, a->Hout, a->Wout, a->stride, a->pad, a->upsample, cfg, a->split_k, a->act, a->residual != nullptr, a->out_f32,
                a->gn_partials ? (a->gn_bwd_x ? 2 : 1) : 0);
    if (asd_cfg_is_ws(cfg)) {
        ASD_CHECK_ARG(asd_conv_ws_ok(a), "weight-streaming convolution: 3x3 stride-1 pad-1 on <= 5 images of 8x8, N % 64 == 0, split_k >= 2, Cin % (32 split_k) == 0");
        hipStream_t sws = (hipStream_t)stream;
        if (asd_conv_ws_launch(a, sws) != ASD_OK) { asd_set_error("weight-streaming convolution: bad image count"); return ASD_ERR_ARG; }
        if (!a->partials_only) asd_launch_splitk_epilogue(a, sws);
        ASD_LAUNCH_CHECK();
        return ASD_OK;
    }
    if (asd_cfg_is_window(cfg)) {
        ASD_CHECK_ARG(asd_cfg_is_pp(cfg) ? asd_conv_pp_ok(a, cfg) : asd_conv_window_ok(a),
                      "window convolution needs a 3x3 stride-1 pad-1 conv with Cin % 64 == 0 (ping-pong: % 32) and H, W % 16 == 0");
        ASD_CHECK_ARG(a->split_k == 1 || a->split_k <= a->Cin / 64, "window convolution: split_k exceeds the channel chunks");
        if (asd_cfg_is_pp(cfg)) {
            ASD_CHECK_ARG(asd_conv_pp_ok(a, cfg), "ping-pong window convolution: image rows % patch rows == 0 and N % tile == 0");
            const int tiles_mp = a->M / bm, tiles_np = a->N / bn;
            if (a->group_m < 1 || a->group_n < 1) asd_pick_group(tiles_mp, tiles_np, bm, bn, asd_conv_pp_lds_bytes(cfg - ASD_GEMM_PP0), &a->group_m, &a->group_n);
            hipStream_t sp = (hipStream_t)stream;
            if (asd_conv_pp_launch(cfg - ASD_GEMM_PP0, a, 8 * asd_div_up(tiles_mp * tiles_np * a->split_k, 8), sp) != ASD_OK) { asd_set_error("bad ping-pong variant"); return ASD_ERR_ARG; }
            if (a->split_k > 1) {
                asd_launch_splitk_epilogue(a, sp);
            }
            ASD_LAUNCH_CHECK();
            return ASD_OK;
        }
        const size_t lds_w = (size_t)2 * 41 * 1024 + (size_t)4 * bn * 128;
        if (a->group_m < 1 || a->group_n < 1)
            asd_pick_group(a->M / 256, asd_div_up(a->N, bn), 256, bn, asd_cfg_is_win2(cfg) ? (size_t)80 * 1024 : lds_w, &a->group_m, &a->group_n);
        const int tiles_w = 8 * asd_div_up((a->M / 256) * asd_div_up(a->N, bn) * a->split_k, 8);
        hipStream_t sw = (hipStream_t)stream;
        if (asd_cfg_is_win2(cfg)) {
            const size_t lds2 = (size_t)41 * 1024 + (size_t)2 * bn * 128;
#define WIN2_LAUNCH(BN_, NW_)                                                                                                          \
    do {                                                                                                                               \
        static std::atomic<unsigned long long> attr_set_devmask{0}; bool attr_set = !asd_attr_needed(attr_set_devmask);                                                                                                  \
        if (!attr_set) {                                                                                                               \
            (void)hipFuncSetAttribute((const void*)conv3x3_win2_kernel<BN_, NW_>, hipFuncAttributeMaxDynamicSharedMemorySize, (int)lds2); \
            attr_set = true;                                                                                                           \
        }                                                                                                                              \
        hipLaunchKernelGGL((conv3x3_win2_kernel<BN_, NW_>), dim3(tiles_w), dim3(NW_ * 64), lds2, sw, *a);                              \
    } while (0)
            if (cfg == 13) WIN2_LAUNCH(64, 4);
            else if (cfg == 14) WIN2_LAUNCH(128, 4);
            else if (bn == 64) WIN2_LAUNCH(64, 8);
            else WIN2_LAUNCH(128, 8);
#undef WIN2_LAUNCH
            if (a->split_k > 1) {
                asd_launch_splitk_epilogue(a, sw);
            }
            ASD_LAUNCH_CHECK();
            return ASD_OK;
        }
        static std::atomic<unsigned long long> attr64_devmask{0}; bool attr64 = !asd_attr_needed(attr64_devmask);static std::atomic<unsigned long long> attr128_devmask{0}; bool attr128 = !asd_attr_needed(attr128_devmask);
        if (bn == 64) {
            if (!attr64) { (void)hipFuncSetAttribute((const void*)conv3x3_win_kernel<64>, hipFuncAttributeMaxDynamicSharedMemorySize, (int)lds_w); attr64 = true; }
            hipLaunchKernelGGL((conv3x3_win_kernel<64>), dim3(tiles_w), dim3(512), lds_w, sw, *a);
        } else {
            if (!attr128) { (void)hipFuncSetAttribute((const void*)conv3x3_win_kernel<128>, hipFuncAttributeMaxDynamicSharedMemorySize, (int)lds_w); attr128 = true; }
            hipLaunchKernelGGL((conv3x3_win_kernel<128>), dim3(tiles_w), dim3(512), lds_w, sw, *a);
        }
        if (a->split_k > 1) {
            asd_launch_splitk_epilogue(a, sw);
        }
        ASD_LAUNCH_CHECK();
        return ASD_OK;
    }
    const int tiles = (a->conv && a->upsample == 3 ? 4 * asd_div_up(a->M / 4, bm) : asd_div_up(a->M, bm)) * asd_div_up(a->N, bn);
    const size_t lds = (size_t)asd_cfg_stages(cfg) * asd_cfg_kgroups(cfg) * (bm + bn) * 128;
    if (a->group_m < 1 || a->group_n < 1) asd_pick_group(asd_div_up(a->M, bm), asd_div_up(a->N, bn), bm, bn, lds, &a->group_m, &a->group_n);
    const dim3 grid(8 * asd_div_up(tiles * a->split_k, 8)), block(asd_gemm_tiles[cfg].wm * asd_gemm_tiles[cfg].wn * asd_cfg_kgroups(cfg) * 64);
    hipStream_t s = (hipStream_t)stream;
#define GEMM_LAUNCH(BM_, BN_, WM_, WN_, CONV_, NST_, KG_, LN_)                                                           \
    do {                                                                                                                 \
        static std::atomic<unsigned long long> attr_set_devmask{0}; bool attr_set = !asd_attr_needed(attr_set_devmask);                                                                                    \
        if (!attr_set) {                                                                                                 \
            (void)hipFuncSetAttribute((const void*)gemm_f16_kernel<BM_, BN_, WM_, WN_, CONV_, NST_, KG_, LN_>,           \
                                      hipFuncAttributeMaxDynamicSharedMemorySize, NST_ * KG_ * (BM_ + BN_) * 128);       \
            attr_set = true;                                                                                             \
        }                                                                                                                \
        hipLaunchKernelGGL((gemm_f16_kernel<BM_, BN_, WM_, WN_, CONV_, NST_, KG_, LN_>), grid, block, lds, s, *a);       \
    } while (0)
#define GEMM_CASE_N(IDX_, BM_, BN_, WM_, WN_, NST_, KG_)                                                                 \
    case IDX_:                                                                                                           \
        if (a->conv) GEMM_LAUNCH(BM_, BN_, WM_, WN_, true, NST_, KG_, false);                                            \
        else if (a->ln_mode == 1) GEMM_LAUNCH(BM_, BN_, WM_, WN_, false, NST_, KG_, true);                               \
        else GEMM_LAUNCH(BM_, BN_, WM_, WN_, false, NST_, KG_, false);                                                   \
        break
#define GEMM_CASE(IDX_, BM_, BN_, WM_, WN_) GEMM_CASE_N(IDX_, BM_, BN_, WM_, WN_, 2, 1)
    switch (cfg) {
        GEMM_CASE(0, 128, 64, 2, 2);
        GEMM_CASE(1, 128, 128, 2, 2);
        GEMM_CASE(2, 256, 64, 4, 2);
        GEMM_CASE(3, 256, 128, 4, 2);
        GEMM_CASE(4, 128, 320, 2, 4);
        GEMM_CASE(5, 256, 256, 2, 4);
        GEMM_CASE(6, 256, 320, 2, 4);
        GEMM_CASE(7, 320, 128, 5, 2);
        GEMM_CASE(12, 64, 64, 2, 2);
        GEMM_CASE_N(15, 64, 64, 2, 2, 4, 1);
        GEMM_CASE_N(16, 64, 64, 2, 2, 2, 2);
        GEMM_CASE_N(17, 64, 64, 2, 2, 2, 4);
        GEMM_CASE_N(18, 128, 64, 2, 2, 2, 2);
        GEMM_CASE_N(19, 128, 128, 2, 2, 2, 2);
        GEMM_CASE_N(26, 128, 64, 2, 2, 6, 1);
        GEMM_CASE_N(27, 64, 64, 2, 2, 8, 1);
        GEMM_CASE_N(28, 128, 128, 2, 2, 4, 1);
        default: asd_set_error("bad tile configuration %d", cfg); return ASD_ERR_ARG;
    }
#undef GEMM_CASE
#undef GEMM_CASE_N
#undef GEMM_LAUNCH
    if (a->split_k > 1 && !a->partials_only) {
        asd_launch_splitk_epilogue(a, s);
    }
    ASD_LAUNCH_CHECK();
    return ASD_OK;
}


static int asd_tune_candidates(const asd_gemm_args* a, int (*out)[2], int max_out) {
    static const int sk_plain[] = {1, 2, 3, 4, 6, 8, 12, 16}, sk_win[] = {1, 2, 3, 4, 5, 6, 8, 10};
    const bool geglu = a->act == 2, window_ok = asd_conv_window_ok(a);
    int n = 0;
    for (int t = 0; t < ASD_GEMM_NCFG && n < max_out; ++t) {
        const int bm = asd_gemm_tiles[t].bm, bn = asd_gemm_tiles[t].bn;
        if (asd_cfg_is_ws(t)) {
            static const int sk_ws[] = {2, 4, 5, 8, 10, 16, 20};
            for (int sk : sk_ws) {
                asd_gemm_args q = *a;
                q.split_k = sk;
                if (!asd_conv_ws_ok(&q) || (a->N / 64) * sk > 512 || (a->N / 64) * sk < 64) continue;
                if (n < max_out) { out[n][0] = t + 1; out[n][1] = sk; ++n; }
            }
            continue;
        }
        if (asd_cfg_is_window(t)) {
            if (asd_cfg_is_pp(t) ? !asd_conv_pp_ok(a, t) : (!window_ok || (bn != 64 && a->N % bn != 0))) continue;
            const int tiles = (a->M / bm) * asd_div_up(a->N, bn);
            for (int sk : sk_win) {
                if (sk > 1 && (a->Cin / 64 < 2 * sk || tiles * sk > 1536)) continue;
                if (n < max_out) { out[n][0] = t + 1; out[n][1] = sk; ++n; }
            }
            continue;
        }
        if (bn != 64 && a->N % bn != 0) continue;
        const bool few = asd_gemm_tiles[t].nst > 2 || asd_gemm_tiles[t].kg > 1;
        if (few && ((a->conv && a->upsample == 2) || (long long)asd_div_up(a->M, bm) * asd_div_up(a->N, bn) > 512 || a->K < 512)) continue;
        if (geglu && (t == 4 || t == 6)) continue;
        if (bn == 64 && a->N % 128 == 0 && a->N >= 256 && bm == 128) continue;
        const int tiles = asd_div_up(a->M, bm) * asd_div_up(a->N, bn);
        for (int sk : sk_plain) {
            if (sk > 1 && (geglu || a->K / sk < 256 || tiles * sk > 1536)) continue;
            if (few && sk != 1 && sk != 2 && sk != 4) continue;
            if (n < max_out) { out[n][0] = t + 1; out[n][1] = sk; ++n; }
        }
    }
    return n;
}

int asd_gemm_tune(const asd_gemm_args* a_in, void* scratch, int64_t scratch_bytes, void* stream) {
    ASD_CHECK_ARG(a_in, "null argument");
    hipStream_t s = (hipStream_t)stream;
    int cand[160][2];
    const int n = asd_tune_candidates(a_in, cand, 160);
    ASD_CHECK_ARG(n > 0, "no tile configuration fits this problem");
    hipEvent_t e0, e1;
    if (hipEventCreate(&e0) != hipSuccess || hipEventCreate(&e1) != hipSuccess) { asd_set_error("hipEventCreate failed"); return ASD_ERR_LAUNCH; }
    float best_ms = 1e30f;
    float ms_of[160];
    static char* cold_flush = nullptr;
    static const size_t cold_bytes = (size_t)320 << 20;
    static const bool want_cold = getenv("ASD_GEMM_TUNE_COLD") && getenv("ASD_GEMM_TUNE_COLD")[0] == '1';
    if (want_cold && !cold_flush && hipMalloc((void**)&cold_flush, cold_bytes) != hipSuccess) cold_flush = nullptr;
    const size_t a_bytes = a_in->conv ? (size_t)(a_in->M / (a_in->Hout * a_in->Wout)) * a_in->Hin * a_in->Win * a_in->Cin * 2
                                      : (size_t)a_in->M * a_in->lda * 2;
    for (int i = 0; i < n; ++i) {
        ms_of[i] = 1e30f;
        asd_gemm_args a = *a_in;
        a.gn_partials = nullptr;
        a.tile_cfg = cand[i][0];
        a.split_k = cand[i][1];
        if (a.split_k > 1) {
            if ((int64_t)a.split_k * a.M * a.N * 4 > scratch_bytes) continue;
            a.workspace = (float*)scratch;
        }
        if (asd_gemm_f16(&a, stream) != ASD_OK) continue;
        float ms = 0.f;
        if (cold_flush) {
            for (int r = 0; r < 4; ++r) {
                (void)hipMemsetAsync(cold_flush, r, cold_bytes, s);
                hipLaunchKernelGGL(asd_touch_kernel, dim3(1024), dim3(256), 0, s, (const uint4*)a.A, a_bytes / 16, (unsigned*)cold_flush);
                hipLaunchKernelGGL(asd_spin_kernel, dim3(1), dim3(1), 0, s, 2000LL);
                hipEventRecord(e0, s);
                asd_gemm_f16(&a, stream);
                hipEventRecord(e1, s);
                hipEventSynchronize(e1);
                float t = 0.f;
                hipEventElapsedTime(&t, e0, e1);
                ms += t;
            }
        } else {
            hipLaunchKernelGGL(asd_spin_kernel, dim3(1), dim3(1), 0, s, 20000LL);
            hipEventRecord(e0, s);
            for (int r = 0; r < 5; ++r) asd_gemm_f16(&a, stream);
            hipEventRecord(e1, s);
            hipEventSynchronize(e1);
            hipEventElapsedTime(&ms, e0, e1);
        }
        ms_of[i] = ms;
        if (ms < best_ms) best_ms = ms;
    }
    hipEventDestroy(e0);
    hipEventDestroy(e1);
    int pick = -1;
    for (int i = 0; i < n; ++i) {
        if (ms_of[i] > 1.04f * best_ms) continue;
        if (pick < 0 || cand[i][1] < cand[pick][1] || (cand[i][1] == cand[pick][1] && ms_of[i] < ms_of[pick])) pick = i;
    }
    if (pick < 0) { asd_set_error("asd_gemm_tune: no candidate ran"); return ASD_ERR_LAUNCH; }
    const asd_plan_key k = asd_plan_key_of(a_in);
    std::lock_guard<std::mutex> lk(g_plans_mu);
    g_plans[k] = asd_plan_val{cand[pick][0], cand[pick][1]};
    ++g_plan_gen;
    return ASD_OK;
}

uint64_t asd_gemm_plan_generation(void) { return g_plan_gen.load(); }

int asd_gemm_plan_entry(int32_t i, int32_t* out11) {
    std::lock_guard<std::mutex> lk(g_plans_mu);
    if (i < 0 || i >= (int)g_plans.size() || !out11) return ASD_ERR_ARG;
    auto it = g_plans.begin();
    std::advance(it, i);
    const asd_plan_key& k = it->first;
    const int32_t v[11] = {k.M, k.N, k.K, k.conv, k.a, k.b, k.c, k.d, k.e, it->second.tile, it->second.split};
    memcpy(out11, v, sizeof(v));
    return ASD_OK;
}

}
```

### scaledreamer_amd/csrc/gemm_tile.h

```cpp
#pragma once
#include "asd_common.h"

typedef _Float16 half_t;
typedef half_t half8 __attribute__((ext_vector_type(8)));
typedef half_t half4 __attribute__((ext_vector_type(4)));
typedef float floatx4 __attribute__((ext_vector_type(4)));

#define GLOBAL_AS __attribute__((address_space(1)))
#define LDS_AS __attribute__((address_space(3)))

__device__ __forceinline__ float gelu_erf(float x) {
    const float z = fabsf(x) * 0.70710678118654752440f;
    const float t = __builtin_amdgcn_rcpf(fmaf(0.3275911f, z, 1.f));
    float poly = fmaf(1.061405429f, t, -1.453152027f);
    poly = fmaf(poly, t, 1.421413741f);
    poly = fmaf(poly, t, -0.284496736f);
    poly = fmaf(poly, t, 0.254829592f);
    const float tail = poly * t * __builtin_amdgcn_exp2f(-1.44269504088896340736f * z * z);
    const float phi = x >= 0.f ? 1.f - 0.5f * tail : 0.5f * tail;
    return x * phi;
}

__device__ __forceinline__ void load_slab(const char* src_row_chunk, char* lds_slab_base) {
    __builtin_amdgcn_global_load_lds((const GLOBAL_AS void*)src_row_chunk, (LDS_AS void*)lds_slab_base, 16, 0, 0);
}

__device__ __forceinline__ bool asd_xcd_item(int bid, int items, int& item) {
    const int per = (items + 7) >> 3;
    item = (bid & 7) * per + (bid >> 3);
    return (bid >> 3) < per && item < items;
}
__device__ __forceinline__ void asd_grouped_tile(int t, int tiles_m, int tiles_n, int gm, int gn, int& tm, int& tn) {
    const int band = t / (gm * tiles_n), r = t - band * gm * tiles_n;
    const int gsz = min(gm, tiles_m - band * gm);
    const int st = r / (gsz * gn), rr = r - st * gsz * gn;
    tm = band * gm + rr % gsz;
    tn = st * gn + rr / gsz;
}

__device__ __forceinline__ float row16_sum(float v) {
    int x;
#define ASD_ROW_ADD(CTRL) x = __builtin_amdgcn_update_dpp(0, __float_as_int(v), CTRL, 0xf, 0xf, true); v += __int_as_float(x)
    ASD_ROW_ADD(0x111); ASD_ROW_ADD(0x112); ASD_ROW_ADD(0x114); ASD_ROW_ADD(0x118);
#undef ASD_ROW_ADD
    return v;
}
__device__ __forceinline__ void gn_tile_begin(float* lds64) {
    __syncthreads();
    if (threadIdx.x < 64) lds64[threadIdx.x] = 0.f;
    __syncthreads();
}
__device__ __forceinline__ float silu_grad_f(float z) {
    const float sg = 1.f / (1.f + __expf(-z));
    return sg * (1.f + z * (1.f - sg));
}
struct GnCol {
    float mean[4], rstd[4], gm[4], bt[4];
};
__device__ __forceinline__ void gn_col_load(const asd_gemm_args& p, int m_any, int n, GnCol& c) {
    if (!p.gn_bwd_x || n >= p.N) return;
    const int b = m_any / p.gn_rows;
    const float inv_cnt = 1.f / ((float)p.gn_rows * (float)p.gn_cg);
    const half4 gm = *(const half4*)((const half_t*)p.gn_bwd_gamma + n), bt = *(const half4*)((const half_t*)p.gn_bwd_beta + n);
#pragma unroll
    for (int r = 0; r < 4; ++r) {
        const int g = (n + r) / p.gn_cg;
        c.mean[r] = p.gn_bwd_fstats[(b * 32 + g) * 2] * inv_cnt;
        c.rstd[r] = rsqrtf(fmaxf(p.gn_bwd_fstats[(b * 32 + g) * 2 + 1] * inv_cnt - c.mean[r] * c.mean[r], 0.f) + p.gn_eps);
        c.gm[r] = (float)gm[r]; c.bt[r] = (float)bt[r];
    }
}
__device__ __forceinline__ void gn_tile_accum(const asd_gemm_args& p, const GnCol& c, const floatx4& o, int m, int n, floatx4& cs, floatx4& cq) {
    if (!p.gn_bwd_x) {
#pragma unroll
        for (int r = 0; r < 4; ++r) { cs[r] += o[r]; cq[r] = fmaf(o[r], o[r], cq[r]); }
        return;
    }
    const half4 xv = *(const half4*)((const half_t*)p.gn_bwd_x + (size_t)m * p.N + n);
#pragma unroll
    for (int r = 0; r < 4; ++r) {
        const float xh = ((float)xv[r] - c.mean[r]) * c.rstd[r];
        float gg = o[r] * c.gm[r];
        if (p.gn_silu) gg *= silu_grad_f(fmaf(xh, c.gm[r], c.bt[r]));
        cs[r] += gg;
        cq[r] = fmaf(gg, xh, cq[r]);
    }
}
__device__ __forceinline__ void gn_tile_flush(float* lds64, floatx4 s, floatx4 q, int n, int N, int cg) {
#pragma unroll
    for (int r = 0; r < 4; ++r) { s[r] = row16_sum(s[r]); q[r] = row16_sum(q[r]); }
    if ((threadIdx.x & 15) == 15) {
#pragma unroll
        for (int r = 0; r < 4; ++r) {
            if (n + r >= N) continue;
            const int g = (n + r) / cg;
            atomicAdd(&lds64[2 * g], s[r]);
            atomicAdd(&lds64[2 * g + 1], q[r]);
        }
    }
}
__device__ __forceinline__ void gn_tile_end(const asd_gemm_args& p, const float* lds64, int record) {
    __syncthreads();
    if (threadIdx.x < 64) p.gn_partials[(size_t)record * 64 + threadIdx.x] = lds64[threadIdx.x];
}

template <int CNT>
__device__ __forceinline__ void ln_fold(const asd_gemm_args& p, float* v, int m, int n, float mean, float rstd) {
    if (p.ln_mode == 1) {
#pragma unroll
        for (int q = 0; q < CNT / 4; ++q) {
            const floatx4 s = *(const floatx4*)(p.ln_sc + n + 4 * q), c = *(const floatx4*)(p.ln_sc + p.N + n + 4 * q);
#pragma unroll
            for (int r = 0; r < 4; ++r) v[4 * q + r] = fmaf(rstd, v[4 * q + r] - mean * s[r], c[r]);
        }
    } else {
        const float s = p.ln_sc[m], c = p.ln_sc[p.M + m];
#pragma unroll
        for (int q = 0; q < CNT / 2; ++q) {
            const floatx4 st = *(const floatx4*)(p.ln_stats + 2 * (n + 2 * q));
            v[2 * q] = fmaf(st[1], v[2 * q] - st[0] * s, c);
            v[2 * q + 1] = fmaf(st[3], v[2 * q + 1] - st[2] * s, c);
        }
    }
}

__device__ __forceinline__ floatx4 gemm_store4(const asd_gemm_args& p, floatx4 v, int m, int n) {
    if (p.bias) {
        const half4 b = *(const half4*)((const half_t*)p.bias + n);
        v[0] += (float)b[0]; v[1] += (float)b[1]; v[2] += (float)b[2]; v[3] += (float)b[3];
    }
    if (p.row_bias) {
        const half4 b = *(const half4*)((const half_t*)p.row_bias + (size_t)(m / p.rows_per_group) * p.ld_row_bias + n);
        v[0] += (float)b[0]; v[1] += (float)b[1]; v[2] += (float)b[2]; v[3] += (float)b[3];
    }
    if (p.act == 1) {
#pragma unroll
        for (int r = 0; r < 4; ++r) v[r] = v[r] / (1.f + __expf(-v[r]));
    }
    if (p.residual) {
        const half4 b = *(const half4*)((const half_t*)p.residual + (size_t)m * p.ldr + n);
        v[0] += (float)b[0]; v[1] += (float)b[1]; v[2] += (float)b[2]; v[3] += (float)b[3];
    }
    if (p.out_f32) {
        *(floatx4*)((float*)p.C + (size_t)m * p.ldc + n) = v;
        return v;
    }
    half4 o = {(half_t)v[0], (half_t)v[1], (half_t)v[2], (half_t)v[3]};
    *(half4*)((half_t*)p.C + (size_t)m * p.ldc + n) = o;
    return floatx4{(float)o[0], (float)o[1], (float)o[2], (float)o[3]};
}

__device__ __forceinline__ int wide_slab_rows(int ws) { return (ws >> 2) * 32 + (ws & 1) * 16 + ((ws >> 1) & 1) * 4; }
__device__ __forceinline__ int wide_lane_row(int lrow) { return (lrow >> 2) * 8 + (lrow & 3); }

__device__ __forceinline__ void gemm_store8(const asd_gemm_args& p, floatx4& lo, floatx4& hi, int m, int n) {
    float v[8] = {lo[0], lo[1], lo[2], lo[3], hi[0], hi[1], hi[2], hi[3]};
    if (p.bias) {
        const half8 b = *(const half8*)((const half_t*)p.bias + n);
#pragma unroll
        for (int k = 0; k < 8; ++k) v[k] += (float)b[k];
    }
    if (p.row_bias) {
        const half8 b = *(const half8*)((const half_t*)p.row_bias + (size_t)(m / p.rows_per_group) * p.ld_row_bias + n);
#pragma unroll
        for (int k = 0; k < 8; ++k) v[k] += (float)b[k];
    }
    if (p.act == 1) {
#pragma unroll
        for (int k = 0; k < 8; ++k) v[k] = v[k] / (1.f + __expf(-v[k]));
    }
    if (p.residual) {
        const half8 b = *(const half8*)((const half_t*)p.residual + (size_t)m * p.ldr + n);
#pragma unroll
        for (int k = 0; k < 8; ++k) v[k] += (float)b[k];
    }
    if (p.out_f32) {
        float* dst = (float*)p.C + (size_t)m * p.ldc + n;
        *(floatx4*)dst = floatx4{v[0], v[1], v[2], v[3]};
        *(floatx4*)(dst + 4) = floatx4{v[4], v[5], v[6], v[7]};
        lo = floatx4{v[0], v[1], v[2], v[3]}; hi = floatx4{v[4], v[5], v[6], v[7]};
        return;
    }
    const half8 o = {(half_t)v[0], (half_t)v[1], (half_t)v[2], (half_t)v[3], (half_t)v[4], (half_t)v[5], (half_t)v[6], (half_t)v[7]};
    *(half8*)((half_t*)p.C + (size_t)m * p.ldc + n) = o;
    lo = floatx4{(float)o[0], (float)o[1], (float)o[2], (float)o[3]}; hi = floatx4{(float)o[4], (float)o[5], (float)o[6], (float)o[7]};
}

template <int TM, int TN, typename RowFn>
__device__ __forceinline__ void tile_epilogue(const asd_gemm_args& p, floatx4 (&acc)[TM][TN], int nb, int kz, int row0, RowFn row, bool gn, float* gn_lds,
                                              const float* ln_mean = nullptr, const float* ln_rstd = nullptr) {
    const int g = (threadIdx.x & 63) >> 4;
    if constexpr (TN % 2 == 0) {
        if (p.wide_rows) {
#pragma unroll
            for (int s2 = 0; s2 < TN / 2; ++s2) {
                const int n = nb + s2 * 32 + g * 8;
                floatx4 cs0 = {0.f, 0.f, 0.f, 0.f}, cq0 = cs0, cs1 = cs0, cq1 = cs0;
#pragma unroll
                for (int i = 0; i < TM; ++i) {
                    const int m = row(i);
                    if (m < 0 || n >= p.N) continue;
                    if (p.split_k > 1) {
                        float* dst = p.workspace + ((size_t)kz * p.M + m) * p.N + n;
                        *(floatx4*)dst = acc[i][2 * s2];
                        *(floatx4*)(dst + 4) = acc[i][2 * s2 + 1];
                    } else {
                        floatx4 lo = acc[i][2 * s2], hi = acc[i][2 * s2 + 1];
                        if (p.ln_mode) {
                            float v8[8] = {lo[0], lo[1], lo[2], lo[3], hi[0], hi[1], hi[2], hi[3]};
                            ln_fold<8>(p, v8, m, n, ln_mean ? ln_mean[i] : 0.f, ln_rstd ? ln_rstd[i] : 0.f);
                            lo = floatx4{v8[0], v8[1], v8[2], v8[3]}; hi = floatx4{v8[4], v8[5], v8[6], v8[7]};
                        }
                        gemm_store8(p, lo, hi, m, n);
                        if (gn) {
#pragma unroll
                            for (int r = 0; r < 4; ++r) {
                                cs0[r] += lo[r]; cq0[r] = fmaf(lo[r], lo[r], cq0[r]);
                                cs1[r] += hi[r]; cq1[r] = fmaf(hi[r], hi[r], cq1[r]);
                            }
                        }
                    }
                }
                if (gn) { gn_tile_flush(gn_lds, cs0, cq0, n, p.N, p.gn_cg); gn_tile_flush(gn_lds, cs1, cq1, n + 4, p.N, p.gn_cg); }
            }
            return;
        }
    }
#pragma unroll
    for (int j = 0; j < TN; ++j) {
        const int n = nb + j * 16 + g * 4;
        floatx4 cs = {0.f, 0.f, 0.f, 0.f}, cq = {0.f, 0.f, 0.f, 0.f};
        GnCol gc;
        if (gn) gn_col_load(p, row0, n, gc);
#pragma unroll
        for (int i = 0; i < TM; ++i) {
            const int m = row(i);
            if (m < 0 || n >= p.N) continue;
            if (p.split_k > 1) *(floatx4*)(p.workspace + ((size_t)kz * p.M + m) * p.N + n) = acc[i][j];
            else {
                floatx4 a4 = acc[i][j];
                if (p.ln_mode) {
                    float v4[4] = {a4[0], a4[1], a4[2], a4[3]};
                    ln_fold<4>(p, v4, m, n, ln_mean ? ln_mean[i] : 0.f, ln_rstd ? ln_rstd[i] : 0.f);
                    a4 = floatx4{v4[0], v4[1], v4[2], v4[3]};
                }
                const floatx4 o = gemm_store4(p, a4, m, n);
                if (gn) gn_tile_accum(p, gc, o, m, n, cs, cq);
            }
        }
        if (gn) gn_tile_flush(gn_lds, cs, cq, n, p.N, p.gn_cg);
    }
}

template <int PER, int MAX>
__device__ __forceinline__ void ring_wait(int ahead) {
    if constexpr (MAX <= 0) {
        asm volatile("s_waitcnt vmcnt(0)" ::: "memory");
    } else {
        if (ahead >= MAX) asm volatile("s_waitcnt vmcnt(%0)" ::"n"(MAX * PER) : "memory");
        else ring_wait<PER, MAX - 1>(ahead);
    }
}
```

### scaledreamer_amd/csrc/nn_ops.hip

```cpp
#include "asd_common.h"

typedef _Float16 half_t;
typedef half_t half8 __attribute__((ext_vector_type(8)));

__device__ __forceinline__ float silu_f(float v) { return v / (1.f + __expf(-v)); }
__device__ __forceinline__ float gelu_f(float x) { return 0.5f * x * (1.f + erff(x * 0.70710678118654752440f)); }

#ifndef GN_UNR
#define GN_UNR 4
#endif
#ifndef GN_CAP_A
#define GN_CAP_A 512
#endif
#ifndef GN_FOLD_RECORDS
#define GN_FOLD_RECORDS 96
#endif

__global__ __launch_bounds__(256) void gn_stats_kernel(const half_t* __restrict__ x1, int c1, const half_t* __restrict__ x2,
                                                       int c2, int hw, int rows_per_block, float* __restrict__ stats) {
    __shared__ float gsum[32], gsq[32];
    const int C = c1 + c2, slots = C / 8, cg = C / 32;
    const int b = blockIdx.x, tid = threadIdx.x;
    if (tid < 32) { gsum[tid] = 0.f; gsq[tid] = 0.f; }
    __syncthreads();
    const int r0 = blockIdx.y * rows_per_block, r1 = min(hw, r0 + rows_per_block);
    const int rows_in_flight = slots >= 256 ? 1 : 256 / slots;
    const int rsub = slots >= 256 ? 0 : tid / slots;
    const int slot0 = slots >= 256 ? tid : tid % slots;
#pragma unroll
    for (int j = 0; j < 2; ++j) {
        const int slot = slot0 + j * 256;
        if (slot >= slots || rsub >= rows_in_flight || (j == 1 && slots <= 256)) continue;
        float s[8], q[8];
#pragma unroll
        for (int k = 0; k < 8; ++k) { s[k] = 0.f; q[k] = 0.f; }
        const int c = slot * 8;
        const half_t* base = c < c1 ? x1 + (size_t)b * hw * c1 + c : x2 + (size_t)b * hw * c2 + (c - c1);
        const size_t rstride = c < c1 ? c1 : c2;
        int r = r0 + rsub;
        for (; r + (GN_UNR - 1) * rows_in_flight < r1; r += GN_UNR * rows_in_flight) {
            half8 v[GN_UNR];
#pragma unroll
            for (int u = 0; u < GN_UNR; ++u) v[u] = *(const half8*)(base + (size_t)(r + u * rows_in_flight) * rstride);
#pragma unroll
            for (int u = 0; u < GN_UNR; ++u)
#pragma unroll
                for (int k = 0; k < 8; ++k) { const float f = (float)v[u][k]; s[k] += f; q[k] = fmaf(f, f, q[k]); }
        }
        for (; r < r1; r += rows_in_flight) {
            const half8 v = *(const half8*)(base + (size_t)r * rstride);
#pragma unroll
            for (int k = 0; k < 8; ++k) { const float f = (float)v[k]; s[k] += f; q[k] = fmaf(f, f, q[k]); }
        }
        int g = c / cg;
        float ss = 0.f, qq = 0.f;
#pragma unroll
        for (int k = 0; k < 8; ++k) {
            const int gk = (c + k) / cg;
            if (gk != g) { atomicAdd(&gsum[g], ss); atomicAdd(&gsq[g], qq); g = gk; ss = 0.f; qq = 0.f; }
            ss += s[k]; qq += q[k];
        }
        atomicAdd(&gsum[g], ss);
        atomicAdd(&gsq[g], qq);
    }
    __syncthreads();
    if (tid < 32) {
        float* part = stats + ((size_t)b * gridDim.y + blockIdx.y) * 64;
        part[tid * 2] = gsum[tid];
        part[tid * 2 + 1] = gsq[tid];
    }
}

__device__ __forceinline__ void gn_reduce_partials(const float* __restrict__ partials, int b, int n_chunks, float* st ,
                                                   float (*scratch)[64] ) {
    const int tid = threadIdx.x, v = tid & 63, q = tid >> 6;
    const float* src = partials + (size_t)b * n_chunks * 64 + v;
    float acc[8];
#pragma unroll
    for (int u = 0; u < 8; ++u) acc[u] = 0.f;
    for (int c = q; c < n_chunks; c += 32) {
        float t[8];
#pragma unroll
        for (int u = 0; u < 8; ++u) t[u] = src[(size_t)min(c + 4 * u, n_chunks - 1) * 64];
#pragma unroll
        for (int u = 0; u < 8; ++u) acc[u] += c + 4 * u < n_chunks ? t[u] : 0.f;
    }
    scratch[q][v] = ((acc[0] + acc[1]) + (acc[2] + acc[3])) + ((acc[4] + acc[5]) + (acc[6] + acc[7]));
    __syncthreads();
    if (tid < 64) st[tid] = (scratch[0][tid] + scratch[1][tid]) + (scratch[2][tid] + scratch[3][tid]);
    __syncthreads();
}

__global__ __launch_bounds__(256) void gn_apply_kernel(const half_t* __restrict__ x1, int c1, const half_t* __restrict__ x2,
                                                       int c2, int hw, int rows_per_block, const half_t* __restrict__ gamma,
                                                       const half_t* __restrict__ beta, float eps, int silu,
                                                       const float* __restrict__ partials, int n_chunks,
                                                       float* __restrict__ stats_out, half_t* __restrict__ y) {
    __shared__ float st[64];
    __shared__ float scratch[4][64];
    const int C = c1 + c2, slots = C / 8, cg = C / 32;
    const int b = blockIdx.x, tid = threadIdx.x;
    const float inv_cnt = 1.f / ((float)hw * (float)cg);
    const int r0 = blockIdx.y * rows_per_block, r1 = min(hw, r0 + rows_per_block);
    const int rows_in_flight = slots >= 256 ? 1 : 256 / slots;
    const int rsub = slots >= 256 ? 0 : tid / slots;
    const int slot0 = slots >= 256 ? tid : tid % slots;
    const bool act0 = slot0 < slots && rsub < rows_in_flight;
    const int cA = slot0 * 8;
    const half_t* baseA = cA < c1 ? x1 + (size_t)b * hw * c1 + cA : x2 + (size_t)b * hw * c2 + (cA - c1);
    const size_t rstrideA = cA < c1 ? c1 : c2;
    half8 pre[GN_UNR], gpre = {}, bpre = {};
    const int rA = r0 + rsub;
    const bool pre_ok = act0 && rA + (GN_UNR - 1) * rows_in_flight < r1;
    if (act0) { gpre = *(const half8*)(gamma + cA); bpre = *(const half8*)(beta + cA); }
    if (pre_ok) {
#pragma unroll
        for (int u = 0; u < GN_UNR; ++u) pre[u] = *(const half8*)(baseA + (size_t)(rA + u * rows_in_flight) * rstrideA);
    }
    gn_reduce_partials(partials, b, n_chunks, st, scratch);
    if (blockIdx.y == 0 && tid < 64) stats_out[b * 64 + tid] = st[tid];
#pragma unroll
    for (int j = 0; j < 2; ++j) {
        const int slot = slot0 + j * 256;
        if (slot >= slots || rsub >= rows_in_flight || (j == 1 && slots <= 256)) continue;
        const int c = slot * 8;
        half8 gv = gpre, bv = bpre;
        if (j == 1) { gv = *(const half8*)(gamma + c); bv = *(const half8*)(beta + c); }
        float sa[8], sb[8];
#pragma unroll
        for (int k = 0; k < 8; ++k) {
            const int g = (c + k) / cg;
            const float mean = st[g * 2] * inv_cnt;
            const float var = fmaxf(st[g * 2 + 1] * inv_cnt - mean * mean, 0.f);
            sa[k] = rsqrtf(var + eps) * (float)gv[k];
            sb[k] = (float)bv[k] - mean * sa[k];
        }
        const half_t* base = c < c1 ? x1 + (size_t)b * hw * c1 + c : x2 + (size_t)b * hw * c2 + (c - c1);
        const size_t rstride = c < c1 ? c1 : c2;
        half_t* ybase = y + (size_t)b * hw * C + c;
        auto emit = [&](const half8& v, int r) __attribute__((always_inline)) {
            half8 o;
#pragma unroll
            for (int k = 0; k < 8; ++k) {
                float f = fmaf((float)v[k], sa[k], sb[k]);
                if (silu) f = silu_f(f);
                o[k] = (half_t)f;
            }
            *(half8*)(ybase + (size_t)r * C) = o;
        };
        int r = r0 + rsub;
        if (j == 0 && pre_ok) {
#pragma unroll
            for (int u = 0; u < GN_UNR; ++u) emit(pre[u], r + u * rows_in_flight);
            r += GN_UNR * rows_in_flight;
        }
        for (; r + (GN_UNR - 1) * rows_in_flight < r1; r += GN_UNR * rows_in_flight) {
            half8 v[GN_UNR];
#pragma unroll
            for (int u = 0; u < GN_UNR; ++u) v[u] = *(const half8*)(base + (size_t)(r + u * rows_in_flight) * rstride);
#pragma unroll
            for (int u = 0; u < GN_UNR; ++u) emit(v[u], r + u * rows_in_flight);
        }
        for (; r < r1; r += rows_in_flight) emit(*(const half8*)(base + (size_t)r * rstride), r);
    }
}

__device__ __forceinline__ float silu_grad(float z) {
    const float sg = 1.f / (1.f + __expf(-z));
    return sg * (1.f + z * (1.f - sg));
}

template <int NT>
__global__ __launch_bounds__(NT) void gn_bwd_stats_kernel(const half_t* __restrict__ x, const half_t* __restrict__ dy, int C,
                                                           int hw, int rows_per_block, const half_t* __restrict__ gamma,
                                                           const half_t* __restrict__ beta, float eps, int silu,
                                                           const float* __restrict__ fstats, float* __restrict__ bstats) {
    __shared__ float gsum[32], gsq[32];
    const int slots = C / 8, cg = C / 32;
    const int b = blockIdx.x, tid = threadIdx.x;
    if (tid < 32) { gsum[tid] = 0.f; gsq[tid] = 0.f; }
    __syncthreads();
    const float inv_cnt = 1.f / ((float)hw * (float)cg);
    const int r0 = blockIdx.y * rows_per_block, r1 = min(hw, r0 + rows_per_block);
    const int rows_in_flight = slots >= NT ? 1 : NT / slots;
    const int rsub = slots >= NT ? 0 : tid / slots;
    const int slot0 = slots >= NT ? tid : tid % slots;
#pragma unroll
    for (int j = 0; j < 2; ++j) {
        const int slot = slot0 + j * NT;
        if (slot >= slots || rsub >= rows_in_flight || (j == 1 && slots <= NT)) continue;
        const int c = slot * 8;
        float mean[8], rstd[8], gm[8], bt[8], s[8], q[8];
#pragma unroll
        for (int k = 0; k < 8; ++k) {
            const int g = (c + k) / cg;
            mean[k] = fstats[(b * 32 + g) * 2] * inv_cnt;
            rstd[k] = rsqrtf(fmaxf(fstats[(b * 32 + g) * 2 + 1] * inv_cnt - mean[k] * mean[k], 0.f) + eps);
            gm[k] = (float)gamma[c + k]; bt[k] = (float)beta[c + k];
            s[k] = 0.f; q[k] = 0.f;
        }
        int r = r0 + rsub;
        for (; r + rows_in_flight < r1; r += 2 * rows_in_flight) {
            const size_t off0 = ((size_t)b * hw + r) * C + c, off1 = off0 + (size_t)rows_in_flight * C;
            const half8 xv0 = *(const half8*)(x + off0), dv0 = *(const half8*)(dy + off0);
            const half8 xv1 = *(const half8*)(x + off1), dv1 = *(const half8*)(dy + off1);
#pragma unroll
            for (int k = 0; k < 8; ++k) {
                const float xh0 = ((float)xv0[k] - mean[k]) * rstd[k], xh1 = ((float)xv1[k] - mean[k]) * rstd[k];
                float g0 = (float)dv0[k] * gm[k], g1 = (float)dv1[k] * gm[k];
                if (silu) { g0 *= silu_grad(fmaf(xh0, gm[k], bt[k])); g1 *= silu_grad(fmaf(xh1, gm[k], bt[k])); }
                s[k] += g0 + g1;
                q[k] = fmaf(g0, xh0, fmaf(g1, xh1, q[k]));
            }
        }
        for (; r < r1; r += rows_in_flight) {
            const size_t off = ((size_t)b * hw + r) * C + c;
            const half8 xv = *(const half8*)(x + off), dv = *(const half8*)(dy + off);
#pragma unroll
            for (int k = 0; k < 8; ++k) {
                const float xh = ((float)xv[k] - mean[k]) * rstd[k];
                float g = (float)dv[k] * gm[k];
                if (silu) g *= silu_grad(fmaf(xh, gm[k], bt[k]));
                s[k] += g;
                q[k] = fmaf(g, xh, q[k]);
            }
        }
        int g = c / cg;
        float ss = 0.f, qq = 0.f;
#pragma unroll
        for (int k = 0; k < 8; ++k) {
            const int gk = (c + k) / cg;
            if (gk != g) { atomicAdd(&gsum[g], ss); atomicAdd(&gsq[g], qq); g = gk; ss = 0.f; qq = 0.f; }
            ss += s[k]; qq += q[k];
        }
        atomicAdd(&gsum[g], ss);
        atomicAdd(&gsq[g], qq);
    }
    __syncthreads();
    if (tid < 32) {
        float* part = bstats + ((size_t)b * gridDim.y + blockIdx.y) * 64;
        part[tid * 2] = gsum[tid];
        part[tid * 2 + 1] = gsq[tid];
    }
}

__global__ __launch_bounds__(256) void gn_bwd_apply_kernel(const half_t* __restrict__ x, const half_t* __restrict__ dy, int C,
                                                           int hw, int rows_per_block, const half_t* __restrict__ gamma,
                                                           const half_t* __restrict__ beta, float eps, int silu,
                                                           const float* __restrict__ fstats, const float* __restrict__ bpartials,
                                                           int n_chunks, const half_t* __restrict__ dx_add,
                                                           half_t* __restrict__ dx) {
    __shared__ float st[64];
    __shared__ float scratch[4][64];
    const int slots = C / 8, cg = C / 32;
    const int b = blockIdx.x, tid = threadIdx.x;
    const float inv_cnt = 1.f / ((float)hw * (float)cg);
    const int r0 = blockIdx.y * rows_per_block, r1 = min(hw, r0 + rows_per_block);
    const int rows_in_flight = slots >= 256 ? 1 : 256 / slots;
    const int rsub = slots >= 256 ? 0 : tid / slots;
    const int slot0 = slots >= 256 ? tid : tid % slots;
    const bool act0 = slot0 < slots && rsub < rows_in_flight;
    const int cA = slot0 * 8, rA = r0 + rsub;
    const bool pre_ok = act0 && rA + rows_in_flight < r1;
    half8 gpre = {}, bpre = {}, px[2], pd[2], pa[2] = {};
    if (act0) { gpre = *(const half8*)(gamma + cA); bpre = *(const half8*)(beta + cA); }
    if (pre_ok) {
#pragma unroll
        for (int u = 0; u < 2; ++u) {
            const size_t off = ((size_t)b * hw + rA + u * rows_in_flight) * C + cA;
            px[u] = *(const half8*)(x + off); pd[u] = *(const half8*)(dy + off);
            if (dx_add) pa[u] = *(const half8*)(dx_add + off);
        }
    }
    gn_reduce_partials(bpartials, b, n_chunks, st, scratch);
#pragma unroll
    for (int j = 0; j < 2; ++j) {
        const int slot = slot0 + j * 256;
        if (slot >= slots || rsub >= rows_in_flight || (j == 1 && slots <= 256)) continue;
        const int c = slot * 8;
        half8 gv = gpre, bv = bpre;
        if (j == 1) { gv = *(const half8*)(gamma + c); bv = *(const half8*)(beta + c); }
        float mean[8], rstd[8], gm[8], bt[8], m1[8], m2[8];
#pragma unroll
        for (int k = 0; k < 8; ++k) {
            const int g = (c + k) / cg;
            mean[k] = fstats[(b * 32 + g) * 2] * inv_cnt;
            rstd[k] = rsqrtf(fmaxf(fstats[(b * 32 + g) * 2 + 1] * inv_cnt - mean[k] * mean[k], 0.f) + eps);
            gm[k] = (float)gv[k]; bt[k] = (float)bv[k];
            m1[k] = st[g * 2] * inv_cnt; m2[k] = st[g * 2 + 1] * inv_cnt;
        }
        auto emit = [&](const half8& xv, const half8& dv, const half8& av, int r) __attribute__((always_inline)) {
            half8 o;
#pragma unroll
            for (int k = 0; k < 8; ++k) {
                const float xh = ((float)xv[k] - mean[k]) * rstd[k];
                float gg = (float)dv[k] * gm[k];
                if (silu) gg *= silu_grad(fmaf(xh, gm[k], bt[k]));
                o[k] = (half_t)(rstd[k] * (gg - m1[k] - xh * m2[k]));
            }
            if (dx_add) {
#pragma unroll
                for (int k = 0; k < 8; ++k) o[k] = (half_t)((float)o[k] + (float)av[k]);
            }
            *(half8*)(dx + ((size_t)b * hw + r) * C + c) = o;
        };
        int r = r0 + rsub;
        if (j == 0 && pre_ok) {
            emit(px[0], pd[0], pa[0], r);
            emit(px[1], pd[1], pa[1], r + rows_in_flight);
            r += 2 * rows_in_flight;
        }
        for (; r + rows_in_flight < r1; r += 2 * rows_in_flight) {
            const size_t off0 = ((size_t)b * hw + r) * C + c, off1 = off0 + (size_t)rows_in_flight * C;
            const half8 xv0 = *(const half8*)(x + off0), dv0 = *(const half8*)(dy + off0);
            const half8 xv1 = *(const half8*)(x + off1), dv1 = *(const half8*)(dy + off1);
            half8 av0 = {}, av1 = {};
            if (dx_add) { av0 = *(const half8*)(dx_add + off0); av1 = *(const half8*)(dx_add + off1); }
            emit(xv0, dv0, av0, r);
            emit(xv1, dv1, av1, r + rows_in_flight);
        }
        for (; r < r1; r += rows_in_flight) {
            const size_t off = ((size_t)b * hw + r) * C + c;
            half8 av = {};
            if (dx_add) av = *(const half8*)(dx_add + off);
            emit(*(const half8*)(x + off), *(const half8*)(dy + off), av, r);
        }
    }
}

__global__ __launch_bounds__(256) void transpose_f16_kernel(const half_t* __restrict__ x, int rows, int cols, int ldx,
                                                            half_t* __restrict__ y, int ldy) {
    __shared__ half_t tile[64][66];
    const int r0 = blockIdx.y * 64, c0 = blockIdx.x * 64;
    for (int q = threadIdx.x; q < 64 * 64; q += 256) {
        const int r = q / 64, c = q % 64;
        tile[r][c] = (r0 + r < rows && c0 + c < cols) ? x[(size_t)(r0 + r) * ldx + c0 + c] : (half_t)0.f;
    }
    __syncthreads();
    for (int q = threadIdx.x; q < 64 * 64; q += 256) {
        const int c = q / 64, r = q % 64;
        if (c0 + c < cols && r0 + r < rows) y[(size_t)(c0 + c) * ldy + r0 + r] = tile[r][c];
    }
}

template <int NV>
__global__ __launch_bounds__(256) void layernorm_kernel(const half_t* __restrict__ x, int rows, int C,
                                                        const half_t* __restrict__ gamma, const half_t* __restrict__ beta,
                                                        float eps, half_t* __restrict__ y) {
    const int lane = threadIdx.x & 63;
    const int wave = blockIdx.x * 4 + (threadIdx.x >> 6), n_waves = gridDim.x * 4;
    half8 gm[NV], bt[NV];
#pragma unroll
    for (int j = 0; j < NV; ++j) {
        const int c = lane * 8 + j * 512;
        if (c < C) { gm[j] = *(const half8*)(gamma + c); bt[j] = *(const half8*)(beta + c); }
    }
    const float inv_c = 1.f / (float)C;
    for (int row = wave; row < rows; row += n_waves) {
        const half_t* xr = x + (size_t)row * C;
        half8 v[NV];
        float s = 0.f;
#pragma unroll
        for (int j = 0; j < NV; ++j) {
            const int c = lane * 8 + j * 512;
            if (c < C) {
                v[j] = *(const half8*)(xr + c);
#pragma unroll
                for (int k = 0; k < 8; ++k) s += (float)v[j][k];
            }
        }
        const float mean = asd_wave_sum(s) * inv_c;
        float q = 0.f;
#pragma unroll
        for (int j = 0; j < NV; ++j)
            if (lane * 8 + j * 512 < C) {
#pragma unroll
                for (int k = 0; k < 8; ++k) { const float d = (float)v[j][k] - mean; q = fmaf(d, d, q); }
            }
        const float rstd = rsqrtf(asd_wave_sum(q) * inv_c + eps);
#pragma unroll
        for (int j = 0; j < NV; ++j) {
            const int c = lane * 8 + j * 512;
            if (c < C) {
                half8 o;
#pragma unroll
                for (int k = 0; k < 8; ++k) o[k] = (half_t)(((float)v[j][k] - mean) * rstd * (float)gm[j][k] + (float)bt[j][k]);
                *(half8*)(y + (size_t)row * C + c) = o;
            }
        }
    }
}


__device__ __forceinline__ float block_reduce(float v, float* red, bool is_max) {
#pragma unroll
    for (int off = 32; off > 0; off >>= 1) {
        const float o = __shfl_xor(v, off, 64);
        v = is_max ? fmaxf(v, o) : v + o;
    }
    const int wave = threadIdx.x >> 6;
    __syncthreads();
    if ((threadIdx.x & 63) == 0) red[wave] = v;
    __syncthreads();
    const float a = red[0], b = red[1], c = red[2], d = red[3];
    return is_max ? fmaxf(fmaxf(a, b), fmaxf(c, d)) : (a + b) + (c + d);
}

template <int NV>
__global__ __launch_bounds__(256) void softmax_kernel(const half_t* __restrict__ x, int ldx, int cols, float scale,
                                                      half_t* __restrict__ y, int ldy) {
    __shared__ float red[4];
    const half_t* xr = x + (size_t)blockIdx.x * ldx;
    half8 v[NV];
    float m = -INFINITY;
#pragma unroll
    for (int j = 0; j < NV; ++j) {
        const int c = threadIdx.x * 8 + j * 2048;
        if (c < cols) {
            v[j] = *(const half8*)(xr + c);
#pragma unroll
            for (int k = 0; k < 8; ++k) m = fmaxf(m, (float)v[j][k]);
        }
    }
    m = block_reduce(m, red, true) * scale;
    float e[NV][8];
    float s = 0.f;
#pragma unroll
    for (int j = 0; j < NV; ++j)
        if (threadIdx.x * 8 + j * 2048 < cols) {
#pragma unroll
            for (int k = 0; k < 8; ++k) { e[j][k] = __expf(fmaf((float)v[j][k], scale, -m)); s += e[j][k]; }
        }
    const float inv = 1.f / block_reduce(s, red, false);
#pragma unroll
    for (int j = 0; j < NV; ++j) {
        const int c = threadIdx.x * 8 + j * 2048;
        if (c < cols) {
            half8 o;
#pragma unroll
            for (int k = 0; k < 8; ++k) o[k] = (half_t)(e[j][k] * inv);
            *(half8*)(y + (size_t)blockIdx.x * ldy + c) = o;
        }
    }
}

template <int NV>
__global__ __launch_bounds__(256) void softmax_bwd_kernel(const half_t* __restrict__ p, const half_t* __restrict__ dp, int ld,
                                                          int cols, float scale, half_t* __restrict__ ds) {
    __shared__ float red[4];
    const size_t base = (size_t)blockIdx.x * ld;
    half8 pv[NV], dv[NV];
    float s = 0.f;
#pragma unroll
    for (int j = 0; j < NV; ++j) {
        const int c = threadIdx.x * 8 + j * 2048;
        if (c < cols) {
            pv[j] = *(const half8*)(p + base + c);
            dv[j] = *(const half8*)(dp + base + c);
#pragma unroll
            for (int k = 0; k < 8; ++k) s = fmaf((float)pv[j][k], (float)dv[j][k], s);
        }
    }
    s = block_reduce(s, red, false);
#pragma unroll
    for (int j = 0; j < NV; ++j) {
        const int c = threadIdx.x * 8 + j * 2048;
        if (c < cols) {
            half8 o;
#pragma unroll
            for (int k = 0; k < 8; ++k) o[k] = (half_t)(scale * (float)pv[j][k] * ((float)dv[j][k] - s));
            *(half8*)(ds + base + c) = o;
        }
    }
}

__global__ __launch_bounds__(256) void geglu_kernel(const half_t* __restrict__ h, int rows, int C, half_t* __restrict__ y) {
    const int slots = C / 8;
    const size_t total = (size_t)rows * slots;
    for (size_t i = (size_t)blockIdx.x * 256 + threadIdx.x; i < total; i += (size_t)gridDim.x * 256) {
        const size_t row = i / slots;
        const int c = (int)(i - row * slots) * 8;
        const half8 a = *(const half8*)(h + row * 2 * C + c), g = *(const half8*)(h + row * 2 * C + C + c);
        half8 o;
#pragma unroll
        for (int k = 0; k < 8; ++k) o[k] = (half_t)((float)a[k] * gelu_f((float)g[k]));
        *(half8*)(y + row * C + c) = o;
    }
}

__global__ __launch_bounds__(256) void silu_kernel(const half_t* __restrict__ x, size_t n8, half_t* __restrict__ y) {
    for (size_t i = (size_t)blockIdx.x * 256 + threadIdx.x; i < n8; i += (size_t)gridDim.x * 256) {
        const half8 v = *(const half8*)(x + i * 8);
        half8 o;
#pragma unroll
        for (int k = 0; k < 8; ++k) o[k] = (half_t)silu_f((float)v[k]);
        *(half8*)(y + i * 8) = o;
    }
}

__global__ void timestep_embedding_kernel(const float* __restrict__ t, int n, int dim, half_t* __restrict__ y) {
    const int i = blockIdx.x * blockDim.x + threadIdx.x;
    const int half = dim / 2;
    if (i >= n * half) return;
    const int r = i / half, k = i - r * half;
    const float freq = expf(-logf(10000.f) * (float)k / (float)half);
    const float a = t[r] * freq;
    y[(size_t)r * dim + k] = (half_t)cosf(a);
    y[(size_t)r * dim + half + k] = (half_t)sinf(a);
}

__global__ __launch_bounds__(256) void concat_kernel(const half_t* __restrict__ x1, int c1, const half_t* __restrict__ x2, int c2,
                                                     size_t rows, half_t* __restrict__ y) {
    const int C = c1 + c2, slots = C / 8;
    const size_t total = rows * slots;
    for (size_t i = (size_t)blockIdx.x * 256 + threadIdx.x; i < total; i += (size_t)gridDim.x * 256) {
        const size_t row = i / slots;
        const int c = (int)(i - row * slots) * 8;
        *(half8*)(y + row * C + c) = c < c1 ? *(const half8*)(x1 + row * c1 + c) : *(const half8*)(x2 + row * c2 + (c - c1));
    }
}

__global__ __launch_bounds__(256) void pad_cast_kernel(const float* __restrict__ x, size_t rows, int c, half_t* __restrict__ y, int c_pad) {
    const size_t total = rows * (size_t)c_pad;
    for (size_t i = (size_t)blockIdx.x * 256 + threadIdx.x; i < total; i += (size_t)gridDim.x * 256) {
        const size_t r = i / c_pad;
        const int j = (int)(i - r * c_pad);
        y[i] = j < c ? (half_t)x[r * c + j] : (half_t)0.f;
    }
}

__global__ __launch_bounds__(1024) void gn_reduce_records_kernel(const float* __restrict__ records, int n, float* __restrict__ out) {
    __shared__ float scratch[16][64];
    const int b = blockIdx.x, S = gridDim.y, per = (n + S - 1) / S;
    const int c0 = blockIdx.y * per, c1 = min(n, c0 + per);
    const int v = threadIdx.x & 63, q = threadIdx.x >> 6;
    const float* src = records + (size_t)b * n * 64 + v;
    float acc[8];
#pragma unroll
    for (int u = 0; u < 8; ++u) acc[u] = 0.f;
    int c = c0 + q;
    for (; c + 7 * 16 < c1; c += 8 * 16) {
        float t[8];
#pragma unroll
        for (int u = 0; u < 8; ++u) t[u] = src[(size_t)(c + u * 16) * 64];
#pragma unroll
        for (int u = 0; u < 8; ++u) acc[u] += t[u];
    }
#pragma unroll
    for (int u = 0; u < 8; ++u)
        if (c + u * 16 < c1) acc[u] += src[(size_t)(c + u * 16) * 64];
    scratch[q][v] = ((acc[0] + acc[1]) + (acc[2] + acc[3])) + ((acc[4] + acc[5]) + (acc[6] + acc[7]));
    __syncthreads();
    if (threadIdx.x < 64) {
        float s = 0.f;
#pragma unroll
        for (int u = 0; u < 16; ++u) s += scratch[u][v];
        out[((size_t)b * S + blockIdx.y) * 64 + v] = s;
    }
}

static int gn_apply_chunks(int hw, int C, int batch) {
    const int slots = C / 8, rif = slots >= 256 ? 1 : 256 / slots;
    const int chunks = asd_div_up(hw, GN_UNR * rif), cap_a = asd_div_up(GN_CAP_A, batch);
    return chunks > cap_a ? cap_a : chunks;
}

__global__ __launch_bounds__(256) void gather_rows_kernel(const uint4* __restrict__ src, const int* __restrict__ idx, size_t row16,
                                                          uint4* __restrict__ dst) {
    const size_t i = blockIdx.y;
    const uint4* s = src + (size_t)idx[i] * row16;
    uint4* d = dst + i * row16;
    for (size_t q = (size_t)blockIdx.x * 256 + threadIdx.x; q < row16; q += (size_t)gridDim.x * 256) d[q] = s[q];
}

extern "C" {

int asd_gather_rows_f16(const void* src, const int32_t* idx_dev, int32_t n_out, int64_t row_halfs, void* dst, void* stream) {
    ASD_CHECK_ARG(src && idx_dev && dst && n_out > 0 && row_halfs > 0 && row_halfs % 8 == 0, "bad argument");
    const size_t row16 = (size_t)row_halfs / 8;
    int bx = (int)((row16 + 1023) / 1024);
    if (bx > 256) bx = 256;
    hipLaunchKernelGGL(gather_rows_kernel, dim3(bx, n_out), dim3(256), 0, (hipStream_t)stream, (const uint4*)src, (const int*)idx_dev, row16,
                       (uint4*)dst);
    ASD_LAUNCH_CHECK();
    return ASD_OK;
}

int asd_groupnorm_f16(const void* x1, int32_t c1, const void* x2, int32_t c2, int32_t batch, int32_t hw, const void* gamma,
                      const void* beta, float eps, int32_t silu, void* y, float* stats, void* stream) {
    ASD_CHECK_ARG(x1 && gamma && beta && y && stats && batch > 0 && hw > 0, "null argument");
    const int C = c1 + (x2 ? c2 : 0);
    if (!x2) c2 = 0;
    ASD_CHECK_ARG(C % 32 == 0 && C % 8 == 0 && c1 % 8 == 0, "channels must be a multiple of 32");
    ASD_CHECK_ARG(((((uintptr_t)gamma) | ((uintptr_t)beta)) & 15) == 0, "gamma / beta must be 16-byte aligned");
    hipStream_t s = (hipStream_t)stream;
    float* partials = stats + 64 * batch;
    int chunks = asd_div_up(hw, 16);
    const int cap_s = asd_div_up(256, batch);
    const int chunks_s = chunks > cap_s ? cap_s : chunks, chunks_a = gn_apply_chunks(hw, C, batch);
    hipLaunchKernelGGL(gn_stats_kernel, dim3(batch, chunks_s), dim3(256), 0, s, (const half_t*)x1, c1, (const half_t*)x2, c2, hw,
                       asd_div_up(hw, chunks_s), partials);
    hipLaunchKernelGGL(gn_apply_kernel, dim3(batch, chunks_a), dim3(256), 0, s, (const half_t*)x1, c1, (const half_t*)x2, c2, hw,
                       asd_div_up(hw, chunks_a), (const half_t*)gamma, (const half_t*)beta, eps, silu, partials, chunks_s, stats,
                       (half_t*)y);
    ASD_LAUNCH_CHECK();
    return ASD_OK;
}

int asd_groupnorm_apply_f16(const void* x, int32_t c, int32_t batch, int32_t hw, const void* gamma, const void* beta, float eps,
                            int32_t silu, const float* partials, int32_t records, void* y, float* stats , void* stream) {
    ASD_CHECK_ARG(x && gamma && beta && y && stats && partials && batch > 0 && hw > 0 && records > 0, "null argument");
    ASD_CHECK_ARG(c % 32 == 0 && c % 8 == 0, "channels must be a multiple of 32");
    ASD_CHECK_ARG(((((uintptr_t)gamma) | ((uintptr_t)beta)) & 15) == 0, "gamma / beta must be 16-byte aligned");
    hipStream_t s = (hipStream_t)stream;
    const int chunks_a = gn_apply_chunks(hw, c, batch);
    const float* part = partials;
    int n = records;
    if (records > GN_FOLD_RECORDS) {
        int slices = asd_div_up(records, 32);
        if (slices > 16) slices = 16;
        float* tmp = stats + 64 * batch;
        hipLaunchKernelGGL(gn_reduce_records_kernel, dim3(batch, slices), dim3(1024), 0, s, partials, records, tmp);
        part = tmp;
        n = slices;
    }
    hipLaunchKernelGGL(gn_apply_kernel, dim3(batch, chunks_a), dim3(256), 0, s, (const half_t*)x, c, (const half_t*)nullptr, 0, hw,
                       asd_div_up(hw, chunks_a), (const half_t*)gamma, (const half_t*)beta, eps, silu, part, n, stats, (half_t*)y);
    ASD_LAUNCH_CHECK();
    return ASD_OK;
}

int asd_groupnorm_bwd_f16(const void* x, const void* dy, int32_t c, int32_t batch, int32_t hw, const void* gamma,
                          const void* beta, float eps, int32_t silu, const float* fwd_stats, const void* dx_add, void* dx,
                          float* bwd_stats, void* stream) {
    ASD_CHECK_ARG(x && dy && gamma && beta && fwd_stats && dx && bwd_stats && batch > 0 && hw > 0, "null argument");
    ASD_CHECK_ARG(c % 32 == 0, "channels must be a multiple of 32");
    ASD_CHECK_ARG(((((uintptr_t)gamma) | ((uintptr_t)beta)) & 15) == 0, "gamma / beta must be 16-byte aligned");
    hipStream_t s = (hipStream_t)stream;
    int chunks = asd_div_up(hw, 16);
    const int cap_s = asd_div_up(256, batch), cap_a = asd_div_up(GN_CAP_A, batch);
    const int chunks_s = chunks > cap_s ? cap_s : chunks, chunks_a = chunks > cap_a ? cap_a : chunks;
    if ((size_t)asd_div_up(hw, chunks_s) * c >= 32768 && c % 8 == 0 && 512 % (c / 8) == 0)
        hipLaunchKernelGGL(gn_bwd_stats_kernel<512>, dim3(batch, chunks_s), dim3(512), 0, s, (const half_t*)x, (const half_t*)dy, c, hw,
                           asd_div_up(hw, chunks_s), (const half_t*)gamma, (const half_t*)beta, eps, silu, fwd_stats, bwd_stats);
    else
        hipLaunchKernelGGL(gn_bwd_stats_kernel<256>, dim3(batch, chunks_s), dim3(256), 0, s, (const half_t*)x, (const half_t*)dy, c, hw,
                           asd_div_up(hw, chunks_s), (const half_t*)gamma, (const half_t*)beta, eps, silu, fwd_stats, bwd_stats);
    hipLaunchKernelGGL(gn_bwd_apply_kernel, dim3(batch, chunks_a), dim3(256), 0, s, (const half_t*)x, (const half_t*)dy, c, hw,
                       asd_div_up(hw, chunks_a), (const half_t*)gamma, (const half_t*)beta, eps, silu, fwd_stats, bwd_stats, chunks_s,
                       (const half_t*)dx_add, (half_t*)dx);
    ASD_LAUNCH_CHECK();
    return ASD_OK;
}

int asd_groupnorm_bwd_apply_f16(const void* x, const void* dy, int32_t c, int32_t batch, int32_t hw, const void* gamma, const void* beta,
                                float eps, int32_t silu, const float* fwd_stats, const float* partials, int32_t records,
                                const void* dx_add, void* dx, float* scratch, void* stream) {
    ASD_CHECK_ARG(x && dy && gamma && beta && fwd_stats && partials && dx && scratch && batch > 0 && hw > 0 && records > 0, "null argument");
    ASD_CHECK_ARG(c % 32 == 0, "channels must be a multiple of 32");
    ASD_CHECK_ARG(((((uintptr_t)gamma) | ((uintptr_t)beta)) & 15) == 0, "gamma / beta must be 16-byte aligned");
    hipStream_t s = (hipStream_t)stream;
    const int chunks = asd_div_up(hw, 16);
    const int cap_a = asd_div_up(GN_CAP_A, batch), chunks_a = chunks > cap_a ? cap_a : chunks;
    const float* part = partials;
    int n = records;
    if (records > GN_FOLD_RECORDS) {
        int slices = asd_div_up(records, 32);
        if (slices > 16) slices = 16;
        hipLaunchKernelGGL(gn_reduce_records_kernel, dim3(batch, slices), dim3(1024), 0, s, partials, records, scratch);
        part = scratch;
        n = slices;
    }
    hipLaunchKernelGGL(gn_bwd_apply_kernel, dim3(batch, chunks_a), dim3(256), 0, s, (const half_t*)x, (const half_t*)dy, c, hw,
                       asd_div_up(hw, chunks_a), (const half_t*)gamma, (const half_t*)beta, eps, silu, fwd_stats, part, n,
                       (const half_t*)dx_add, (half_t*)dx);
    ASD_LAUNCH_CHECK();
    return ASD_OK;
}

int asd_transpose_f16(const void* x, int32_t rows, int32_t cols, int32_t ldx, void* y, int32_t ldy, void* stream) {
    ASD_CHECK_ARG(x && y && rows > 0 && cols > 0 && ldx >= cols && ldy >= rows, "bad argument");
    hipLaunchKernelGGL(transpose_f16_kernel, dim3(asd_div_up(cols, 64), asd_div_up(rows, 64)), dim3(256), 0, (hipStream_t)stream,
                       (const half_t*)x, rows, cols, ldx, (half_t*)y, ldy);
    ASD_LAUNCH_CHECK();
    return ASD_OK;
}

int asd_layernorm_f16(const void* x, int32_t rows, int32_t c, const void* gamma, const void* beta, float eps, void* y,
                      void* stream) {
    ASD_CHECK_ARG(x && gamma && beta && y && rows > 0, "null argument");
    ASD_CHECK_ARG(c % 8 == 0 && c <= 2048, "channels must be a multiple of 8 and <= 2048");
    int blocks = asd_div_up(rows, 4);
    if (blocks > 2048) blocks = 2048;
    const dim3 g(blocks), blk(256);
    hipStream_t s = (hipStream_t)stream;
#define LN_LAUNCH(NV) hipLaunchKernelGGL((layernorm_kernel<NV>), g, blk, 0, s, (const half_t*)x, rows, c, (const half_t*)gamma, \
                                         (const half_t*)beta, eps, (half_t*)y)
    if (c <= 512) LN_LAUNCH(1);
    else if (c <= 1024) LN_LAUNCH(2);
    else if (c <= 1536) LN_LAUNCH(3);
    else LN_LAUNCH(4);
#undef LN_LAUNCH
    ASD_LAUNCH_CHECK();
    return ASD_OK;
}

int asd_softmax_f16(const void* x, int32_t ldx, int32_t rows, int32_t cols, float scale, void* y, int32_t ldy, void* stream) {
    ASD_CHECK_ARG(x && y && rows > 0 && cols > 0, "null argument");
    ASD_CHECK_ARG(cols % 8 == 0 && cols <= 8192 && ldx % 8 == 0 && ldy % 8 == 0, "cols must be a multiple of 8 and <= 8192");
    const dim3 g(rows), blk(256);
    hipStream_t s = (hipStream_t)stream;
#define SM_LAUNCH(NV) hipLaunchKernelGGL((softmax_kernel<NV>), g, blk, 0, s, (const half_t*)x, ldx, cols, scale, (half_t*)y, ldy)
    if (cols <= 2048) SM_LAUNCH(1);
    else if (cols <= 4096) SM_LAUNCH(2);
    else SM_LAUNCH(4);
#undef SM_LAUNCH
    ASD_LAUNCH_CHECK();
    return ASD_OK;
}

int asd_softmax_bwd_f16(const void* p, const void* dp, int32_t ld, int32_t rows, int32_t cols, float scale, void* ds,
                        void* stream) {
    ASD_CHECK_ARG(p && dp && ds && rows > 0 && cols > 0, "null argument");
    ASD_CHECK_ARG(cols % 8 == 0 && cols <= 8192 && ld % 8 == 0, "cols must be a multiple of 8 and <= 8192");
    const dim3 g(rows), blk(256);
    hipStream_t s = (hipStream_t)stream;
#define SMB_LAUNCH(NV) hipLaunchKernelGGL((softmax_bwd_kernel<NV>), g, blk, 0, s, (const half_t*)p, (const half_t*)dp, ld, cols, scale, (half_t*)ds)
    if (cols <= 2048) SMB_LAUNCH(1);
    else if (cols <= 4096) SMB_LAUNCH(2);
    else SMB_LAUNCH(4);
#undef SMB_LAUNCH
    ASD_LAUNCH_CHECK();
    return ASD_OK;
}

int asd_geglu_f16(const void* h, int32_t rows, int32_t c, void* y, void* stream) {
    ASD_CHECK_ARG(h && y && rows > 0 && c % 8 == 0, "bad argument");
    hipLaunchKernelGGL(geglu_kernel, dim3(asd_grid_for((size_t)rows * c / 8, 256)), dim3(256), 0, (hipStream_t)stream,
                       (const half_t*)h, rows, c, (half_t*)y);
    ASD_LAUNCH_CHECK();
    return ASD_OK;
}

int asd_silu_f16(const void* x, int64_t n, void* y, void* stream) {
    ASD_CHECK_ARG(x && y && n > 0 && n % 8 == 0, "bad argument");
    hipLaunchKernelGGL(silu_kernel, dim3(asd_grid_for(n / 8, 256)), dim3(256), 0, (hipStream_t)stream, (const half_t*)x,
                       (size_t)(n / 8), (half_t*)y);
    ASD_LAUNCH_CHECK();
    return ASD_OK;
}

int asd_timestep_embedding_f16(const float* t, int32_t n, int32_t dim, void* y, void* stream) {
    ASD_CHECK_ARG(t && y && n > 0 && dim % 2 == 0, "bad argument");
    hipLaunchKernelGGL(timestep_embedding_kernel, dim3(asd_div_up(n * dim / 2, 256)), dim3(256), 0, (hipStream_t)stream, t, n,
                       dim, (half_t*)y);
    ASD_LAUNCH_CHECK();
    return ASD_OK;
}

int asd_concat_f16(const void* x1, int32_t c1, const void* x2, int32_t c2, int64_t rows, void* y, void* stream) {
    ASD_CHECK_ARG(x1 && x2 && y && rows > 0 && c1 % 8 == 0 && c2 % 8 == 0, "bad argument");
    hipLaunchKernelGGL(concat_kernel, dim3(asd_grid_for((size_t)rows * (c1 + c2) / 8, 256)), dim3(256), 0, (hipStream_t)stream,
                       (const half_t*)x1, c1, (const half_t*)x2, c2, (size_t)rows, (half_t*)y);
    ASD_LAUNCH_CHECK();
    return ASD_OK;
}

int asd_pad_cast_f16(const float* x, int32_t rows, int32_t c, void* y, int32_t c_pad, void* stream) {
    ASD_CHECK_ARG(x && y && rows > 0 && c > 0 && c_pad >= c, "bad argument");
    const size_t total = (size_t)rows * c_pad;
    hipLaunchKernelGGL(pad_cast_kernel, dim3(asd_grid_for(total, 256)), dim3(256), 0, (hipStream_t)stream, x, (size_t)rows, c, (half_t*)y, c_pad);
    ASD_LAUNCH_CHECK();
    return ASD_OK;
}

}
```

Measured before the change: 71.91 steps/s.

## Use fast exp2/rcp SiLU and template GroupNorm kernels on silu/add flags

Replaces the SiLU and SiLU-gradient math in the GEMM epilogues and GroupNorm kernels with hardware exp2 and reciprocal intrinsics, with the log2e scale folded into the per-channel affine coefficients. The GroupNorm apply, backward-stats and backward-apply kernels are templated on the silu and dx_add flags, so those runtime branches disappear. The backward loops are unrolled four rows deep using a generic unroll-trip helper, and the inverse count is computed on the host. The aim is fewer transcendental and divide instructions plus more loads in flight in memory-bound normalization passes, at the cost of slightly lower-precision sigmoid results and more kernel instantiations.

```diff
diff --git a/scaledreamer_amd/csrc/asd_common.h b/scaledreamer_amd/csrc/asd_common.h
--- a/scaledreamer_amd/csrc/asd_common.h
+++ b/scaledreamer_amd/csrc/asd_common.h
@@ -100,6 +100,13 @@
 __device__ __forceinline__ float asd_softplus(float x) { return x > 20.f ? x : log1pf(expf(x)); }
 __device__ __forceinline__ float asd_sigmoid(float x) { return 1.f / (1.f + expf(-x)); }
 __device__ __forceinline__ float asd_clampf(float v, float lo, float hi) { return v < lo ? lo : (v > hi ? hi : v); }
+
+#define ASD_NEG_LOG2E (-1.4426950408889634f)
+__device__ __forceinline__ float asd_sigmoid_exp2(float t) { return __builtin_amdgcn_rcpf(1.f + __builtin_amdgcn_exp2f(t)); }
+__device__ __forceinline__ float asd_sigmoid_fast(float z) { return asd_sigmoid_exp2(ASD_NEG_LOG2E * z); }
+__device__ __forceinline__ float asd_silu_fast(float z) { return z * asd_sigmoid_fast(z); }
+__device__ __forceinline__ float asd_silu_grad_s(float z, float s) { return fmaf(z, fmaf(-s, s, s), s); }
+__device__ __forceinline__ float asd_silu_grad_fast(float z) { return asd_silu_grad_s(z, asd_sigmoid_fast(z)); }
 
 __device__ __forceinline__ uint32_t asd_grid_index(const asd_grid_meta& m, int l, uint32_t cx, uint32_t cy,
                                                    uint32_t cz) {
diff --git a/scaledreamer_amd/csrc/gemm.hip b/scaledreamer_amd/csrc/gemm.hip
--- a/scaledreamer_amd/csrc/gemm.hip
+++ b/scaledreamer_amd/csrc/gemm.hip
@@ -720,7 +720,7 @@
     }
     if (p.act == 1) {
 #pragma unroll
-        for (int r = 0; r < 4; ++r) v[r] = v[r] / (1.f + __expf(-v[r]));
+        for (int r = 0; r < 4; ++r) v[r] = asd_silu_fast(v[r]);
     }
     if (p.residual) {
         const half4 b = *(const half4*)((const half_t*)p.residual + (size_t)m * p.ldr + n);
@@ -771,7 +771,7 @@
         }
         if (p.act == 1) {
 #pragma unroll
-            for (int r = 0; r < 4; ++r) w[r] = w[r] / (1.f + __expf(-w[r]));
+            for (int r = 0; r < 4; ++r) w[r] = asd_silu_fast(w[r]);
         }
         if (p.residual) {
             const half4 b = *(const half4*)((const half_t*)p.residual + (size_t)m * p.ldr + n);
@@ -794,7 +794,7 @@
 
 #define GNA_THREADS 1024
 template <int NV>
-__global__ __launch_bounds__(GNA_THREADS) void splitk_epilogue_gnapply_kernel(const asd_gemm_args p, int splits) {
+__global__ __launch_bounds__(GNA_THREADS) void splitk_epilogue_gnapply_kernel(const asd_gemm_args p, int splits, float inv_cnt ) {
     __shared__ float red[2 * (GNA_THREADS / 64)];
     const int cg = p.gn_cg, g4 = cg >> 2, rows = p.gn_rows;
     const int b = blockIdx.x >> 5, g = blockIdx.x & 31;
@@ -846,7 +846,7 @@
         for (int r = 0; r < 4; ++r) w[r] += (float)rbias[i][r];
         if (p.act == 1) {
 #pragma unroll
-            for (int r = 0; r < 4; ++r) w[r] = w[r] / (1.f + __expf(-w[r]));
+            for (int r = 0; r < 4; ++r) w[r] = asd_silu_fast(w[r]);
         }
 #pragma unroll
         for (int r = 0; r < 4; ++r) w[r] += (float)resid[i][r];
@@ -868,7 +868,6 @@
 #pragma unroll
     for (int w = 0; w < GNA_THREADS / 64; ++w) { sum += red[2 * w]; sq += red[2 * w + 1]; }
     if (p.gn_apply_stats && tid == 0) { p.gn_apply_stats[b * 64 + g * 2] = sum; p.gn_apply_stats[b * 64 + g * 2 + 1] = sq; }
-    const float inv_cnt = 1.f / ((float)rows * (float)cg);
     const float mean = sum * inv_cnt;
     const float var = fmaxf(sq * inv_cnt - mean * mean, 0.f);
     const float rstd = rsqrtf(var + p.gn_apply_eps);
@@ -882,7 +881,7 @@
         for (int r = 0; r < 4; ++r) {
             const float sa = rstd * (float)gm[r];
             float f = fmaf(v[i][r], sa, (float)bt[r] - mean * sa);
-            if (p.gn_apply_silu) f = f / (1.f + __expf(-f));
+            if (p.gn_apply_silu) f = asd_silu_fast(f);
             o[r] = (half_t)f;
         }
         *(half4*)((half_t*)p.gn_apply_y + (size_t)m * p.N + n) = o;
@@ -904,9 +903,10 @@
     const int nv = a->gn_apply_y ? asd_gemm_gn_apply_nv(a) : 0;
     if (nv > 0) {
         const dim3 grid((a->M / a->gn_rows) * 32);
-        if (nv == 1) hipLaunchKernelGGL(splitk_epilogue_gnapply_kernel<1>, grid, dim3(GNA_THREADS), 0, s, *a, a->split_k);
-        else if (nv == 3) hipLaunchKernelGGL(splitk_epilogue_gnapply_kernel<3>, grid, dim3(GNA_THREADS), 0, s, *a, a->split_k);
-        else hipLaunchKernelGGL(splitk_epilogue_gnapply_kernel<ASD_GNAPPLY_MAX_NV>, grid, dim3(GNA_THREADS), 0, s, *a, a->split_k);
+        const float inv_cnt = 1.f / ((float)a->gn_rows * (float)a->gn_cg);
+        if (nv == 1) hipLaunchKernelGGL(splitk_epilogue_gnapply_kernel<1>, grid, dim3(GNA_THREADS), 0, s, *a, a->split_k, inv_cnt);
+        else if (nv == 3) hipLaunchKernelGGL(splitk_epilogue_gnapply_kernel<3>, grid, dim3(GNA_THREADS), 0, s, *a, a->split_k, inv_cnt);
+        else hipLaunchKernelGGL(splitk_epilogue_gnapply_kernel<ASD_GNAPPLY_MAX_NV>, grid, dim3(GNA_THREADS), 0, s, *a, a->split_k, inv_cnt);
         return;
     }
     const size_t total4 = (size_t)a->M * a->N / 4;
diff --git a/scaledreamer_amd/csrc/gemm_tile.h b/scaledreamer_amd/csrc/gemm_tile.h
--- a/scaledreamer_amd/csrc/gemm_tile.h
+++ b/scaledreamer_amd/csrc/gemm_tile.h
@@ -50,10 +50,7 @@
     if (threadIdx.x < 64) lds64[threadIdx.x] = 0.f;
     __syncthreads();
 }
-__device__ __forceinline__ float silu_grad_f(float z) {
-    const float sg = 1.f / (1.f + __expf(-z));
-    return sg * (1.f + z * (1.f - sg));
-}
+__device__ __forceinline__ float silu_grad_f(float z) { return asd_silu_grad_fast(z); }
 struct GnCol {
     float mean[4], rstd[4], gm[4], bt[4];
 };
@@ -135,7 +132,7 @@
     }
     if (p.act == 1) {
 #pragma unroll
-        for (int r = 0; r < 4; ++r) v[r] = v[r] / (1.f + __expf(-v[r]));
+        for (int r = 0; r < 4; ++r) v[r] = asd_silu_fast(v[r]);
     }
     if (p.residual) {
         const half4 b = *(const half4*)((const half_t*)p.residual + (size_t)m * p.ldr + n);
@@ -167,7 +164,7 @@
     }
     if (p.act == 1) {
 #pragma unroll
-        for (int k = 0; k < 8; ++k) v[k] = v[k] / (1.f + __expf(-v[k]));
+        for (int k = 0; k < 8; ++k) v[k] = asd_silu_fast(v[k]);
     }
     if (p.residual) {
         const half8 b = *(const half8*)((const half_t*)p.residual + (size_t)m * p.ldr + n);
diff --git a/scaledreamer_amd/csrc/nn_ops.hip b/scaledreamer_amd/csrc/nn_ops.hip
--- a/scaledreamer_amd/csrc/nn_ops.hip
+++ b/scaledreamer_amd/csrc/nn_ops.hip
@@ -1,9 +1,10 @@
 #include "asd_common.h"
+#include <type_traits>
 
 typedef _Float16 half_t;
 typedef half_t half8 __attribute__((ext_vector_type(8)));
 
-__device__ __forceinline__ float silu_f(float v) { return v / (1.f + __expf(-v)); }
+__device__ __forceinline__ float silu_f(float v) { return asd_silu_fast(v); }
 __device__ __forceinline__ float gelu_f(float x) { return 0.5f * x * (1.f + erff(x * 0.70710678118654752440f)); }
 
 #ifndef GN_UNR
@@ -91,16 +92,16 @@
     __syncthreads();
 }
 
+template <bool SILU>
 __global__ __launch_bounds__(256) void gn_apply_kernel(const half_t* __restrict__ x1, int c1, const half_t* __restrict__ x2,
                                                        int c2, int hw, int rows_per_block, const half_t* __restrict__ gamma,
-                                                       const half_t* __restrict__ beta, float eps, int silu,
+                                                       const half_t* __restrict__ beta, float eps, float inv_cnt,
                                                        const float* __restrict__ partials, int n_chunks,
                                                        float* __restrict__ stats_out, half_t* __restrict__ y) {
     __shared__ float st[64];
     __shared__ float scratch[4][64];
     const int C = c1 + c2, slots = C / 8, cg = C / 32;
     const int b = blockIdx.x, tid = threadIdx.x;
-    const float inv_cnt = 1.f / ((float)hw * (float)cg);
     const int r0 = blockIdx.y * rows_per_block, r1 = min(hw, r0 + rows_per_block);
     const int rows_in_flight = slots >= 256 ? 1 : 256 / slots;
     const int rsub = slots >= 256 ? 0 : tid / slots;
@@ -126,7 +127,7 @@
         const int c = slot * 8;
         half8 gv = gpre, bv = bpre;
         if (j == 1) { gv = *(const half8*)(gamma + c); bv = *(const half8*)(beta + c); }
-        float sa[8], sb[8];
+        float sa[8], sb[8], ta[8], tb[8];
 #pragma unroll
         for (int k = 0; k < 8; ++k) {
             const int g = (c + k) / cg;
@@ -134,6 +135,7 @@
             const float var = fmaxf(st[g * 2 + 1] * inv_cnt - mean * mean, 0.f);
             sa[k] = rsqrtf(var + eps) * (float)gv[k];
             sb[k] = (float)bv[k] - mean * sa[k];
+            ta[k] = ASD_NEG_LOG2E * sa[k]; tb[k] = ASD_NEG_LOG2E * sb[k];
         }
         const half_t* base = c < c1 ? x1 + (size_t)b * hw * c1 + c : x2 + (size_t)b * hw * c2 + (c - c1);
         const size_t rstride = c < c1 ? c1 : c2;
@@ -142,8 +144,9 @@
             half8 o;
 #pragma unroll
             for (int k = 0; k < 8; ++k) {
-                float f = fmaf((float)v[k], sa[k], sb[k]);
-                if (silu) f = silu_f(f);
+                const float xf = (float)v[k];
+                float f = fmaf(xf, sa[k], sb[k]);
+                if (SILU) f *= asd_sigmoid_exp2(fmaf(xf, ta[k], tb[k]));
                 o[k] = (half_t)f;
             }
             *(half8*)(ybase + (size_t)r * C) = o;
@@ -154,33 +157,40 @@
             for (int u = 0; u < GN_UNR; ++u) emit(pre[u], r + u * rows_in_flight);
             r += GN_UNR * rows_in_flight;
         }
-        for (; r + (GN_UNR - 1) * rows_in_flight < r1; r += GN_UNR * rows_in_flight) {
-            half8 v[GN_UNR];
-#pragma unroll
-            for (int u = 0; u < GN_UNR; ++u) v[u] = *(const half8*)(base + (size_t)(r + u * rows_in_flight) * rstride);
-#pragma unroll
-            for (int u = 0; u < GN_UNR; ++u) emit(v[u], r + u * rows_in_flight);
-        }
-        for (; r < r1; r += rows_in_flight) emit(*(const half8*)(base + (size_t)r * rstride), r);
-    }
-}
-
-__device__ __forceinline__ float silu_grad(float z) {
-    const float sg = 1.f / (1.f + __expf(-z));
-    return sg * (1.f + z * (1.f - sg));
-}
-
-template <int NT>
+        auto trips = [&](auto uc) __attribute__((always_inline)) {
+            constexpr int U = decltype(uc)::value;
+            for (; r + (U - 1) * rows_in_flight < r1; r += U * rows_in_flight) {
+                half8 v[U];
+#pragma unroll
+                for (int u = 0; u < U; ++u) v[u] = *(const half8*)(base + (size_t)(r + u * rows_in_flight) * rstride);
+#pragma unroll
+                for (int u = 0; u < U; ++u) emit(v[u], r + u * rows_in_flight);
+            }
+        };
+        trips(std::integral_constant<int, GN_UNR>{});
+        trips(std::integral_constant<int, 1>{});
+    }
+}
+
+__device__ __forceinline__ float silu_grad(float z) { return asd_silu_grad_fast(z); }
+
+#ifndef GN_BWD_UNR
+#define GN_BWD_UNR 4
+#endif
+#ifndef GN_BWD_WIDE_NT
+#define GN_BWD_WIDE_NT 512
+#endif
+
+template <int NT, bool SILU>
 __global__ __launch_bounds__(NT) void gn_bwd_stats_kernel(const half_t* __restrict__ x, const half_t* __restrict__ dy, int C,
                                                            int hw, int rows_per_block, const half_t* __restrict__ gamma,
-                                                           const half_t* __restrict__ beta, float eps, int silu,
+                                                           const half_t* __restrict__ beta, float eps, float inv_cnt,
                                                            const float* __restrict__ fstats, float* __restrict__ bstats) {
     __shared__ float gsum[32], gsq[32];
     const int slots = C / 8, cg = C / 32;
     const int b = blockIdx.x, tid = threadIdx.x;
     if (tid < 32) { gsum[tid] = 0.f; gsq[tid] = 0.f; }
     __syncthreads();
-    const float inv_cnt = 1.f / ((float)hw * (float)cg);
     const int r0 = blockIdx.y * rows_per_block, r1 = min(hw, r0 + rows_per_block);
     const int rows_in_flight = slots >= NT ? 1 : NT / slots;
     const int rsub = slots >= NT ? 0 : tid / slots;
@@ -190,41 +200,43 @@
         const int slot = slot0 + j * NT;
         if (slot >= slots || rsub >= rows_in_flight || (j == 1 && slots <= NT)) continue;
         const int c = slot * 8;
-        float mean[8], rstd[8], gm[8], bt[8], s[8], q[8];
+        float rstd[8], nmr[8], gm[8], bt[8], s[8], q[8];
 #pragma unroll
         for (int k = 0; k < 8; ++k) {
             const int g = (c + k) / cg;
-            mean[k] = fstats[(b * 32 + g) * 2] * inv_cnt;
-            rstd[k] = rsqrtf(fmaxf(fstats[(b * 32 + g) * 2 + 1] * inv_cnt - mean[k] * mean[k], 0.f) + eps);
+            const float mean = fstats[(b * 32 + g) * 2] * inv_cnt;
+            rstd[k] = rsqrtf(fmaxf(fstats[(b * 32 + g) * 2 + 1] * inv_cnt - mean * mean, 0.f) + eps);
+            nmr[k] = -mean * rstd[k];
             gm[k] = (float)gamma[c + k]; bt[k] = (float)beta[c + k];
             s[k] = 0.f; q[k] = 0.f;
         }
-        int r = r0 + rsub;
-        for (; r + rows_in_flight < r1; r += 2 * rows_in_flight) {
-            const size_t off0 = ((size_t)b * hw + r) * C + c, off1 = off0 + (size_t)rows_in_flight * C;
-            const half8 xv0 = *(const half8*)(x + off0), dv0 = *(const half8*)(dy + off0);
-            const half8 xv1 = *(const half8*)(x + off1), dv1 = *(const half8*)(dy + off1);
+        auto accum = [&](const half8& xv, const half8& dv) __attribute__((always_inline)) {
 #pragma unroll
             for (int k = 0; k < 8; ++k) {
-                const float xh0 = ((float)xv0[k] - mean[k]) * rstd[k], xh1 = ((float)xv1[k] - mean[k]) * rstd[k];
-                float g0 = (float)dv0[k] * gm[k], g1 = (float)dv1[k] * gm[k];
-                if (silu) { g0 *= silu_grad(fmaf(xh0, gm[k], bt[k])); g1 *= silu_grad(fmaf(xh1, gm[k], bt[k])); }
-                s[k] += g0 + g1;
-                q[k] = fmaf(g0, xh0, fmaf(g1, xh1, q[k]));
-            }
-        }
-        for (; r < r1; r += rows_in_flight) {
-            const size_t off = ((size_t)b * hw + r) * C + c;
-            const half8 xv = *(const half8*)(x + off), dv = *(const half8*)(dy + off);
-#pragma unroll
-            for (int k = 0; k < 8; ++k) {
-                const float xh = ((float)xv[k] - mean[k]) * rstd[k];
+                const float xh = fmaf((float)xv[k], rstd[k], nmr[k]);
                 float g = (float)dv[k] * gm[k];
-                if (silu) g *= silu_grad(fmaf(xh, gm[k], bt[k]));
+                if (SILU) g *= silu_grad(fmaf(xh, gm[k], bt[k]));
                 s[k] += g;
                 q[k] = fmaf(g, xh, q[k]);
             }
-        }
+        };
+        int r = r0 + rsub;
+        auto trips = [&](auto uc) __attribute__((always_inline)) {
+            constexpr int U = decltype(uc)::value;
+            for (; r + (U - 1) * rows_in_flight < r1; r += U * rows_in_flight) {
+                half8 xv[U], dv[U];
+#pragma unroll
+                for (int u = 0; u < U; ++u) {
+                    const size_t off = ((size_t)b * hw + r + u * rows_in_flight) * C + c;
+                    xv[u] = *(const half8*)(x + off); dv[u] = *(const half8*)(dy + off);
+                }
+#pragma unroll
+                for (int u = 0; u < U; ++u) accum(xv[u], dv[u]);
+            }
+        };
+        trips(std::integral_constant<int, GN_BWD_UNR>{});
+        if (GN_BWD_UNR > 2) trips(std::integral_constant<int, 2>{});
+        trips(std::integral_constant<int, 1>{});
         int g = c / cg;
         float ss = 0.f, qq = 0.f;
 #pragma unroll
@@ -244,9 +256,10 @@
     }
 }
 
+template <bool SILU, bool ADD>
 __global__ __launch_bounds__(256) void gn_bwd_apply_kernel(const half_t* __restrict__ x, const half_t* __restrict__ dy, int C,
                                                            int hw, int rows_per_block, const half_t* __restrict__ gamma,
-                                                           const half_t* __restrict__ beta, float eps, int silu,
+                                                           const half_t* __restrict__ beta, float eps, float inv_cnt,
                                                            const float* __restrict__ fstats, const float* __restrict__ bpartials,
                                                            int n_chunks, const half_t* __restrict__ dx_add,
                                                            half_t* __restrict__ dx) {
@@ -254,7 +267,6 @@
     __shared__ float scratch[4][64];
     const int slots = C / 8, cg = C / 32;
     const int b = blockIdx.x, tid = threadIdx.x;
-    const float inv_cnt = 1.f / ((float)hw * (float)cg);
     const int r0 = blockIdx.y * rows_per_block, r1 = min(hw, r0 + rows_per_block);
     const int rows_in_flight = slots >= 256 ? 1 : 256 / slots;
     const int rsub = slots >= 256 ? 0 : tid / slots;
@@ -269,7 +281,7 @@
         for (int u = 0; u < 2; ++u) {
             const size_t off = ((size_t)b * hw + rA + u * rows_in_flight) * C + cA;
             px[u] = *(const half8*)(x + off); pd[u] = *(const half8*)(dy + off);
-            if (dx_add) pa[u] = *(const half8*)(dx_add + off);
+            if (ADD) pa[u] = *(const half8*)(dx_add + off);
         }
     }
     gn_reduce_partials(bpartials, b, n_chunks, st, scratch);
@@ -280,27 +292,26 @@
         const int c = slot * 8;
         half8 gv = gpre, bv = bpre;
         if (j == 1) { gv = *(const half8*)(gamma + c); bv = *(const half8*)(beta + c); }
-        float mean[8], rstd[8], gm[8], bt[8], m1[8], m2[8];
+        float rstd[8], nmr[8], gm[8], bt[8], G[8], c1[8], c2[8];
 #pragma unroll
         for (int k = 0; k < 8; ++k) {
             const int g = (c + k) / cg;
-            mean[k] = fstats[(b * 32 + g) * 2] * inv_cnt;
-            rstd[k] = rsqrtf(fmaxf(fstats[(b * 32 + g) * 2 + 1] * inv_cnt - mean[k] * mean[k], 0.f) + eps);
+            const float mean = fstats[(b * 32 + g) * 2] * inv_cnt;
+            rstd[k] = rsqrtf(fmaxf(fstats[(b * 32 + g) * 2 + 1] * inv_cnt - mean * mean, 0.f) + eps);
+            nmr[k] = -mean * rstd[k];
             gm[k] = (float)gv[k]; bt[k] = (float)bv[k];
-            m1[k] = st[g * 2] * inv_cnt; m2[k] = st[g * 2 + 1] * inv_cnt;
+            G[k] = gm[k] * rstd[k];
+            c1[k] = -(st[g * 2] * inv_cnt) * rstd[k]; c2[k] = -(st[g * 2 + 1] * inv_cnt) * rstd[k];
         }
         auto emit = [&](const half8& xv, const half8& dv, const half8& av, int r) __attribute__((always_inline)) {
             half8 o;
 #pragma unroll
             for (int k = 0; k < 8; ++k) {
-                const float xh = ((float)xv[k] - mean[k]) * rstd[k];
-                float gg = (float)dv[k] * gm[k];
-                if (silu) gg *= silu_grad(fmaf(xh, gm[k], bt[k]));
-                o[k] = (half_t)(rstd[k] * (gg - m1[k] - xh * m2[k]));
-            }
-            if (dx_add) {
-#pragma unroll
-                for (int k = 0; k < 8; ++k) o[k] = (half_t)((float)o[k] + (float)av[k]);
+                const float xh = fmaf((float)xv[k], rstd[k], nmr[k]);
+                const float lin = fmaf(xh, c2[k], c1[k]);
+                float f = SILU ? fmaf((float)dv[k] * G[k], silu_grad(fmaf(xh, gm[k], bt[k])), lin) : fmaf((float)dv[k], G[k], lin);
+                if (ADD) f += (float)av[k];
+                o[k] = (half_t)f;
             }
             *(half8*)(dx + ((size_t)b * hw + r) * C + c) = o;
         };
@@ -310,21 +321,23 @@
             emit(px[1], pd[1], pa[1], r + rows_in_flight);
             r += 2 * rows_in_flight;
         }
-        for (; r + rows_in_flight < r1; r += 2 * rows_in_flight) {
-            const size_t off0 = ((size_t)b * hw + r) * C + c, off1 = off0 + (size_t)rows_in_flight * C;
-            const half8 xv0 = *(const half8*)(x + off0), dv0 = *(const half8*)(dy + off0);
-            const half8 xv1 = *(const half8*)(x + off1), dv1 = *(const half8*)(dy + off1);
-            half8 av0 = {}, av1 = {};
-            if (dx_add) { av0 = *(const half8*)(dx_add + off0); av1 = *(const half8*)(dx_add + off1); }
-            emit(xv0, dv0, av0, r);
-            emit(xv1, dv1, av1, r + rows_in_flight);
-        }
-        for (; r < r1; r += rows_in_flight) {
-            const size_t off = ((size_t)b * hw + r) * C + c;
-            half8 av = {};
-            if (dx_add) av = *(const half8*)(dx_add + off);
-            emit(*(const half8*)(x + off), *(const half8*)(dy + off), av, r);
-        }
+        auto trips = [&](auto uc) __attribute__((always_inline)) {
+            constexpr int U = decltype(uc)::value;
+            for (; r + (U - 1) * rows_in_flight < r1; r += U * rows_in_flight) {
+                half8 xv[U], dv[U], av[U] = {};
+#pragma unroll
+                for (int u = 0; u < U; ++u) {
+                    const size_t off = ((size_t)b * hw + r + u * rows_in_flight) * C + c;
+                    xv[u] = *(const half8*)(x + off); dv[u] = *(const half8*)(dy + off);
+                    if (ADD) av[u] = *(const half8*)(dx_add + off);
+                }
+#pragma unroll
+                for (int u = 0; u < U; ++u) emit(xv[u], dv[u], av[u], r + u * rows_in_flight);
+            }
+        };
+        trips(std::integral_constant<int, GN_BWD_UNR>{});
+        if (GN_BWD_UNR > 2) trips(std::integral_constant<int, 2>{});
+        trips(std::integral_constant<int, 1>{});
     }
 }
 
@@ -571,6 +584,47 @@
     const uint4* s = src + (size_t)idx[i] * row16;
     uint4* d = dst + i * row16;
     for (size_t q = (size_t)blockIdx.x * 256 + threadIdx.x; q < row16; q += (size_t)gridDim.x * 256) d[q] = s[q];
+}
+
+static void gn_launch_apply(dim3 grid, hipStream_t s, const void* x1, int c1, const void* x2, int c2, int hw, int rows_per_block,
+                            const void* gamma, const void* beta, float eps, int silu, const float* partials, int n_chunks, float* stats,
+                            void* y) {
+    const float inv_cnt = 1.f / ((float)hw * (float)((c1 + c2) / 32));
+#define GN_APPLY_ARGS (const half_t*)x1, c1, (const half_t*)x2, c2, hw, rows_per_block, (const half_t*)gamma, (const half_t*)beta, eps, inv_cnt, \
+                      partials, n_chunks, stats, (half_t*)y
+    if (silu) hipLaunchKernelGGL(gn_apply_kernel<true>, grid, dim3(256), 0, s, GN_APPLY_ARGS);
+    else hipLaunchKernelGGL(gn_apply_kernel<false>, grid, dim3(256), 0, s, GN_APPLY_ARGS);
+#undef GN_APPLY_ARGS
+}
+
+static void gn_launch_bwd_stats(bool wide, dim3 grid, hipStream_t s, const void* x, const void* dy, int c, int hw, int rows_per_block,
+                                const void* gamma, const void* beta, float eps, int silu, const float* fstats, float* bstats) {
+    const float inv_cnt = 1.f / ((float)hw * (float)(c / 32));
+#define GN_BWD_STATS_ARGS (const half_t*)x, (const half_t*)dy, c, hw, rows_per_block, (const half_t*)gamma, (const half_t*)beta, eps, inv_cnt, fstats, bstats
+    if (wide) {
+        if (silu) hipLaunchKernelGGL((gn_bwd_stats_kernel<GN_BWD_WIDE_NT, true>), grid, dim3(GN_BWD_WIDE_NT), 0, s, GN_BWD_STATS_ARGS);
+        else hipLaunchKernelGGL((gn_bwd_stats_kernel<GN_BWD_WIDE_NT, false>), grid, dim3(GN_BWD_WIDE_NT), 0, s, GN_BWD_STATS_ARGS);
+    } else {
+        if (silu) hipLaunchKernelGGL((gn_bwd_stats_kernel<256, true>), grid, dim3(256), 0, s, GN_BWD_STATS_ARGS);
+        else hipLaunchKernelGGL((gn_bwd_stats_kernel<256, false>), grid, dim3(256), 0, s, GN_BWD_STATS_ARGS);
+    }
+#undef GN_BWD_STATS_ARGS
+}
+
+static void gn_launch_bwd_apply(dim3 grid, hipStream_t s, const void* x, const void* dy, int c, int hw, int rows_per_block, const void* gamma,
+                                const void* beta, float eps, int silu, const float* fstats, const float* bpartials, int n_chunks,
+                                const void* dx_add, void* dx) {
+    const float inv_cnt = 1.f / ((float)hw * (float)(c / 32));
+#define GN_BWD_APPLY_ARGS (const half_t*)x, (const half_t*)dy, c, hw, rows_per_block, (const half_t*)gamma, (const half_t*)beta, eps, inv_cnt, fstats, \
+                          bpartials, n_chunks, (const half_t*)dx_add, (half_t*)dx
+    if (silu) {
+        if (dx_add) hipLaunchKernelGGL((gn_bwd_apply_kernel<true, true>), grid, dim3(256), 0, s, GN_BWD_APPLY_ARGS);
+        else hipLaunchKernelGGL((gn_bwd_apply_kernel<true, false>), grid, dim3(256), 0, s, GN_BWD_APPLY_ARGS);
+    } else {
+        if (dx_add) hipLaunchKernelGGL((gn_bwd_apply_kernel<false, true>), grid, dim3(256), 0, s, GN_BWD_APPLY_ARGS);
+        else hipLaunchKernelGGL((gn_bwd_apply_kernel<false, false>), grid, dim3(256), 0, s, GN_BWD_APPLY_ARGS);
+    }
+#undef GN_BWD_APPLY_ARGS
 }
 
 extern "C" {
@@ -600,9 +654,7 @@
     const int chunks_s = chunks > cap_s ? cap_s : chunks, chunks_a = gn_apply_chunks(hw, C, batch);
     hipLaunchKernelGGL(gn_stats_kernel, dim3(batch, chunks_s), dim3(256), 0, s, (const half_t*)x1, c1, (const half_t*)x2, c2, hw,
                        asd_div_up(hw, chunks_s), partials);
-    hipLaunchKernelGGL(gn_apply_kernel, dim3(batch, chunks_a), dim3(256), 0, s, (const half_t*)x1, c1, (const half_t*)x2, c2, hw,
-                       asd_div_up(hw, chunks_a), (const half_t*)gamma, (const half_t*)beta, eps, silu, partials, chunks_s, stats,
-                       (half_t*)y);
+    gn_launch_apply(dim3(batch, chunks_a), s, x1, c1, x2, c2, hw, asd_div_up(hw, chunks_a), gamma, beta, eps, silu, partials, chunks_s, stats, y);
     ASD_LAUNCH_CHECK();
     return ASD_OK;
 }
@@ -624,8 +676,7 @@
         part = tmp;
         n = slices;
     }
-    hipLaunchKernelGGL(gn_apply_kernel, dim3(batch, chunks_a), dim3(256), 0, s, (const half_t*)x, c, (const half_t*)nullptr, 0, hw,
-                       asd_div_up(hw, chunks_a), (const half_t*)gamma, (const half_t*)beta, eps, silu, part, n, stats, (half_t*)y);
+    gn_launch_apply(dim3(batch, chunks_a), s, x, c, nullptr, 0, hw, asd_div_up(hw, chunks_a), gamma, beta, eps, silu, part, n, stats, y);
     ASD_LAUNCH_CHECK();
     return ASD_OK;
 }
@@ -640,15 +691,10 @@
     int chunks = asd_div_up(hw, 16);
     const int cap_s = asd_div_up(256, batch), cap_a = asd_div_up(GN_CAP_A, batch);
     const int chunks_s = chunks > cap_s ? cap_s : chunks, chunks_a = chunks > cap_a ? cap_a : chunks;
-    if ((size_t)asd_div_up(hw, chunks_s) * c >= 32768 && c % 8 == 0 && 512 % (c / 8) == 0)
-        hipLaunchKernelGGL(gn_bwd_stats_kernel<512>, dim3(batch, chunks_s), dim3(512), 0, s, (const half_t*)x, (const half_t*)dy, c, hw,
-                           asd_div_up(hw, chunks_s), (const half_t*)gamma, (const half_t*)beta, eps, silu, fwd_stats, bwd_stats);
-    else
-        hipLaunchKernelGGL(gn_bwd_stats_kernel<256>, dim3(batch, chunks_s), dim3(256), 0, s, (const half_t*)x, (const half_t*)dy, c, hw,
-                           asd_div_up(hw, chunks_s), (const half_t*)gamma, (const half_t*)beta, eps, silu, fwd_stats, bwd_stats);
-    hipLaunchKernelGGL(gn_bwd_apply_kernel, dim3(batch, chunks_a), dim3(256), 0, s, (const half_t*)x, (const half_t*)dy, c, hw,
-                       asd_div_up(hw, chunks_a), (const half_t*)gamma, (const half_t*)beta, eps, silu, fwd_stats, bwd_stats, chunks_s,
-                       (const half_t*)dx_add, (half_t*)dx);
+    const bool wide = (size_t)asd_div_up(hw, chunks_s) * c >= 32768 && c % 8 == 0 && GN_BWD_WIDE_NT % (c / 8) == 0;
+    gn_launch_bwd_stats(wide, dim3(batch, chunks_s), s, x, dy, c, hw, asd_div_up(hw, chunks_s), gamma, beta, eps, silu, fwd_stats, bwd_stats);
+    gn_launch_bwd_apply(dim3(batch, chunks_a), s, x, dy, c, hw, asd_div_up(hw, chunks_a), gamma, beta, eps, silu, fwd_stats, bwd_stats, chunks_s,
+                        dx_add, dx);
     ASD_LAUNCH_CHECK();
     return ASD_OK;
 }
@@ -671,9 +717,7 @@
         part = scratch;
         n = slices;
     }
-    hipLaunchKernelGGL(gn_bwd_apply_kernel, dim3(batch, chunks_a), dim3(256), 0, s, (const half_t*)x, (const half_t*)dy, c, hw,
-                       asd_div_up(hw, chunks_a), (const half_t*)gamma, (const half_t*)beta, eps, silu, fwd_stats, part, n,
-                       (const half_t*)dx_add, (half_t*)dx);
+    gn_launch_bwd_apply(dim3(batch, chunks_a), s, x, dy, c, hw, asd_div_up(hw, chunks_a), gamma, beta, eps, silu, fwd_stats, part, n, dx_add, dx);
     ASD_LAUNCH_CHECK();
     return ASD_OK;
 }
```

Measured after the change: 73.04 steps/s, median of 6. 1.6% higher.
